# akamiru/bce

Hardware: NVIDIA B200
Metric: compress_MBps_bwt_cse (higher is better)
Workload: dtype u8/u32

## Files before the change

### bce_b200/csrc/api.cu

```cuda
#include <stdarg.h>
#include <stdlib.h>

#include <algorithm>
#include <chrono>
#include <new>

#include "ctx.h"

namespace bce {

static bool g_trace = false;
bool trace_on() { return g_trace; }
static void refresh_trace() {
  const char* v = getenv("BCE_GPU_TRACE");
  g_trace = v && *v && *v != '0';
}

void set_error(Ctx* c, const char* fmt, ...) {
  if (!c) return;
  va_list ap;
  va_start(ap, fmt);
  vsnprintf(c->err, sizeof c->err, fmt, ap);
  va_end(ap);
}

int DevBuf::ensure(Ctx* c, size_t bytes) {
  if (bytes <= cap && p) return BCE_GPU_OK;
  if (p) { cudaFree(p); p = nullptr; cap = 0; }
  size_t want = (bytes + (size_t(1) << 20) - 1) & ~((size_t(1) << 20) - 1);
  cudaError_t e = cudaMalloc(&p, want);
  if (e != cudaSuccess) {
    p = nullptr;
    cudaGetLastError();
    set_error(c, "cudaMalloc(%zu bytes) failed: %s", want, cudaGetErrorString(e));
    return BCE_GPU_E_NOMEM;
  }
  e = cudaMemsetAsync(p, 0, want, c->stream);
  if (e != cudaSuccess) { set_error(c, "cudaMemset failed: %s", cudaGetErrorString(e)); return BCE_GPU_E_CUDA; }
  cap = want;
  return BCE_GPU_OK;
}
void DevBuf::release() {
  if (p) cudaFree(p);
  p = nullptr; cap = 0;
}
int PinnedBuf::ensure(Ctx* c, size_t bytes) {
  if (bytes <= cap && p) return BCE_GPU_OK;
  if (p) { cudaFreeHost(p); p = nullptr; cap = 0; }
  size_t want = (bytes + (size_t(1) << 20) - 1) & ~((size_t(1) << 20) - 1);
  cudaError_t e = cudaHostAlloc(&p, want, cudaHostAllocDefault);
  if (e != cudaSuccess) {
    p = nullptr;
    cudaGetLastError();
    set_error(c, "cudaHostAlloc(%zu bytes) failed: %s", want, cudaGetErrorString(e));
    return BCE_GPU_E_NOMEM;
  }
  cap = want;
  return BCE_GPU_OK;
}
void PinnedBuf::release() {
  if (p) cudaFreeHost(p);
  p = nullptr; cap = 0;
}

int next_tag(Ctx* c) {
  if (++c->desc_tag >= 0x3FFFFFFFu) {
    c->desc_tag = 1;
    if (c->desc.p) cudaMemsetAsync(c->desc.p, 0, c->desc.cap, c->stream);
  }
  return int(c->desc_tag);
}

constexpr size_t kStageChunk = size_t(64) << 20;
bool is_pinned(const void* p) {
  cudaPointerAttributes at;
  if (cudaPointerGetAttributes(&at, p) != cudaSuccess) { cudaGetLastError(); return false; }
  return at.type == cudaMemoryTypeHost;
}
int h2d(Ctx* c, void* dst, const void* src, size_t bytes) {
  if (!bytes) return BCE_GPU_OK;
  if (is_pinned(src) || bytes <= (size_t(1) << 20)) {
    BCE_CUDA(c, cudaMemcpyAsync(dst, src, bytes, cudaMemcpyHostToDevice, c->stream));
    BCE_CUDA(c, cudaStreamSynchronize(c->stream));
    return BCE_GPU_OK;
  }
  BCE_TRY(c->pinned_io.ensure(c, 2 * kStageChunk));
  char* stage = c->pinned_io.as<char>();
  cudaEvent_t done[2] = {c->ev[6], c->ev[7]};
  bool used[2] = {false, false};
  size_t at = 0;
  for (int b = 0; at < bytes; b ^= 1) {
    size_t len = bytes - at < kStageChunk ? bytes - at : kStageChunk;
    if (used[b]) BCE_CUDA(c, cudaEventSynchronize(done[b]));
    memcpy(stage + b * kStageChunk, static_cast<const char*>(src) + at, len);
    BCE_CUDA(c, cudaMemcpyAsync(static_cast<char*>(dst) + at, stage + b * kStageChunk, len,
                                cudaMemcpyHostToDevice, c->stream));
    BCE_CUDA(c, cudaEventRecord(done[b], c->stream));
    used[b] = true;
    at += len;
  }
  BCE_CUDA(c, cudaStreamSynchronize(c->stream));
  return BCE_GPU_OK;
}
int d2h(Ctx* c, void* dst, const void* src, size_t bytes) {
  if (!bytes) return BCE_GPU_OK;
  if (is_pinned(dst) || bytes <= (size_t(1) << 20)) {
    BCE_CUDA(c, cudaMemcpyAsync(dst, src, bytes, cudaMemcpyDeviceToHost, c->stream));
    BCE_CUDA(c, cudaStreamSynchronize(c->stream));
    return BCE_GPU_OK;
  }
  BCE_TRY(c->pinned_io.ensure(c, 2 * kStageChunk));
  char* stage = c->pinned_io.as<char>();
  cudaEvent_t done[2] = {c->ev[6], c->ev[7]};
  size_t at = 0, pending_at[2] = {0, 0}, pending_len[2] = {0, 0};
  bool used[2] = {false, false};
  for (int b = 0; at < bytes; b ^= 1) {
    size_t len = bytes - at < kStageChunk ? bytes - at : kStageChunk;
    if (used[b]) {
      BCE_CUDA(c, cudaEventSynchronize(done[b]));
      memcpy(static_cast<char*>(dst) + pending_at[b], stage + b * kStageChunk, pending_len[b]);
    }
    BCE_CUDA(c, cudaMemcpyAsync(stage + b * kStageChunk, static_cast<const char*>(src) + at, len,
                                cudaMemcpyDeviceToHost, c->stream));
    BCE_CUDA(c, cudaEventRecord(done[b], c->stream));
    used[b] = true; pending_at[b] = at; pending_len[b] = len;
    at += len;
  }
  BCE_CUDA(c, cudaStreamSynchronize(c->stream));
  int order[2] = {0, 1};
  if (used[0] && used[1] && pending_at[1] < pending_at[0]) { order[0] = 1; order[1] = 0; }
  for (int k = 0; k < 2; ++k) {
    int b = order[k];
    if (used[b]) memcpy(static_cast<char*>(dst) + pending_at[b], stage + b * kStageChunk, pending_len[b]);
  }
  return BCE_GPU_OK;
}

size_t scratch_budget(Ctx* c) {
  size_t b = size_t(double(c->total_mem) * 0.70);
  if (c->scratch_limit && c->scratch_limit < b) b = c->scratch_limit;
  return b;
}

static int check_n(Ctx* c, uint32_t n) {
  if (n == 0 || n >= 0x80000000u) { set_error(c, "n = %u outside 1 .. 2^31-1", n); return BCE_GPU_E_ARG; }
  return BCE_GPU_OK;
}

static void begin_call(Ctx* c) {
  refresh_trace();
  c->err[0] = 0;
  cudaSetDevice(c->device);
}

static int upload_text(Ctx* c, const uint8_t* T, uint32_t n) {
  if (c->prefetch_pending) {
    c->prefetch_pending = false;
    const bool arrived = cudaEventQuery(c->ev_prefetch[1]) == cudaSuccess;
    BCE_CUDA(c, cudaEventSynchronize(c->ev_prefetch[1]));
    BCE_TRACE("prefetched input: %s, %s", arrived ? "already on the device" : "still in flight",
              (c->prefetch_src == T && c->prefetch_n == n) ? "adopted" : "another input: discarded");
    if (c->prefetch_src == T && c->prefetch_n == n) {
      float ms = 0;
      BCE_CUDA(c, cudaEventElapsedTime(&ms, c->ev_prefetch[0], c->ev_prefetch[1]));
      c->stats.ms_h2d += ms;
      c->n = n;
      c->text_resident = true;
      c->bwt_resident = false;
      c->ranks_resident = false;
      return BCE_GPU_OK;
    }
  }
  BCE_TRY(c->text.ensure(c, size_t(n) + 128));
  cudaEvent_t a = c->ev[4], b = c->ev[5];
  BCE_CUDA(c, cudaEventRecord(a, c->stream));
  BCE_TRY(h2d(c, c->text.p, T, n));
  BCE_CUDA(c, cudaEventRecord(b, c->stream));
  BCE_CUDA(c, cudaEventSynchronize(b));
  float ms = 0;
  BCE_CUDA(c, cudaEventElapsedTime(&ms, a, b));
  c->stats.ms_h2d += ms;
  c->n = n;
  c->text_resident = true;
  c->bwt_resident = false;
  c->ranks_resident = false;
  return BCE_GPU_OK;
}

static int run_bwt(Ctx* c, uint32_t n, uint32_t* sa_host) {
  cudaEvent_t a = c->ev[4], b = c->ev[5];
  BCE_CUDA(c, cudaEventRecord(a, c->stream));
  BCE_TRY(suffix_sort_bwt(c, n, sa_host));
  BCE_CUDA(c, cudaEventRecord(b, c->stream));
  BCE_CUDA(c, cudaEventSynchronize(b));
  float ms = 0;
  BCE_CUDA(c, cudaEventElapsedTime(&ms, a, b));
  c->stats.ms_bwt_total += ms;
  return BCE_GPU_OK;
}

static int run_cse_begin(Ctx* c, uint32_t n) {
  c->cse_emit_mode_active = int(c->emit_mode);
  cudaEvent_t a = c->ev[4], b = c->ev[5];
  BCE_CUDA(c, cudaEventRecord(a, c->stream));
  BCE_TRY(wavelet_build(c, n));
  BCE_TRY(cse_begin(c, n));
  BCE_CUDA(c, cudaEventRecord(b, c->stream));
  BCE_CUDA(c, cudaEventSynchronize(b));
  float ms = 0;
  BCE_CUDA(c, cudaEventElapsedTime(&ms, a, b));
  c->stats.ms_cse_total += ms;
  return BCE_GPU_OK;
}

static void reset_stats(Ctx* c, uint32_t n) {
  memset(&c->stats, 0, sizeof c->stats);
  c->stats.n = n;
}

}

using bce::Ctx;

extern "C" {

int bce_gpu_abi_version(void) { return BCE_GPU_ABI_VERSION; }

const char* bce_gpu_error_string(int code) {
  switch (code) {
    case BCE_GPU_OK: return "ok";
    case BCE_GPU_E_ARG: return "bad argument";
    case BCE_GPU_E_NOMEM: return "out of memory";
    case BCE_GPU_E_CUDA: return "CUDA failure";
    case BCE_GPU_E_STATE: return "call sequence violated";
    case BCE_GPU_E_FRONTIER: return "CSE frontier exceeded its device memory";
    case BCE_GPU_E_INTERNAL: return "internal consistency check failed";
    case BCE_GPU_E_NODEVICE: return "no usable CUDA device";
    default: return "unknown error";
  }
}

int bce_gpu_open(int device, bce_gpu_ctx** out) {
  if (!out) return BCE_GPU_E_ARG;
  *out = nullptr;
  int count = 0;
  if (cudaGetDeviceCount(&count) != cudaSuccess || count == 0) { cudaGetLastError(); return BCE_GPU_E_NODEVICE; }
  if (device < 0 || device >= count) return BCE_GPU_E_ARG;
  if (cudaSetDevice(device) != cudaSuccess) { cudaGetLastError(); return BCE_GPU_E_NODEVICE; }
  cudaDeviceProp prop;
  if (cudaGetDeviceProperties(&prop, device) != cudaSuccess) { cudaGetLastError(); return BCE_GPU_E_CUDA; }
  if (prop.major < 10 || !prop.cooperativeLaunch) return BCE_GPU_E_NODEVICE;
  Ctx* c = new (std::nothrow) Ctx();
  if (!c) return BCE_GPU_E_NOMEM;
  c->device = device;
  c->sm_count = prop.multiProcessorCount;
  c->total_mem = prop.totalGlobalMem;
  bool ok = cudaStreamCreateWithFlags(&c->stream, cudaStreamNonBlocking) == cudaSuccess &&
            cudaStreamCreateWithFlags(&c->copy_stream, cudaStreamNonBlocking) == cudaSuccess &&
            cudaStreamCreateWithFlags(&c->h2d_stream, cudaStreamNonBlocking) == cudaSuccess &&
            cudaEventCreate(&c->ev_prefetch[0]) == cudaSuccess && cudaEventCreate(&c->ev_prefetch[1]) == cudaSuccess;
  for (int i = 0; ok && i < 8; ++i) ok = cudaEventCreate(&c->ev[i]) == cudaSuccess;
  for (int i = 0; ok && i < 256; ++i) ok = cudaEventCreate(&c->pass_ev[i]) == cudaSuccess;
  if (ok) ok = bce::radix_init_device(c) == BCE_GPU_OK;
  if (ok) ok = c->small.ensure(c, bce::kSmallBytes) == BCE_GPU_OK;
  if (ok) ok = c->pinned_small.ensure(c, bce::kSmallBytes) == BCE_GPU_OK;
  if (ok) ok = cudaStreamSynchronize(c->stream) == cudaSuccess;
  if (!ok) { bce_gpu_close(c); return BCE_GPU_E_CUDA; }
  *out = c;
  return BCE_GPU_OK;
}

void bce_gpu_close(bce_gpu_ctx* h) {
  if (!h) return;
  Ctx* c = static_cast<Ctx*>(h);
  cudaSetDevice(c->device);
  if (c->stream) cudaStreamSynchronize(c->stream);
  bce::cse_destroy(c);
  c->text.release(); c->bwt.release(); c->ranks.release(); c->scratch.release();
  c->small.release(); c->desc.release();
  c->scan_tmp.release(); c->pack_tmp.release();
  c->pinned_small.release(); c->pinned_emit.release(); c->pinned_emit2.release(); c->pinned_io.release();
  c->pinned_many.release(); c->pinned_many2.release();
  for (auto& e : c->ev) if (e) cudaEventDestroy(e);
  for (auto& e : c->pass_ev) if (e) cudaEventDestroy(e);
  if (c->stream) cudaStreamDestroy(c->stream);
  if (c->copy_stream) cudaStreamDestroy(c->copy_stream);
  if (c->h2d_stream) { cudaStreamSynchronize(c->h2d_stream); cudaStreamDestroy(c->h2d_stream); }
  for (auto& e : c->ev_prefetch) if (e) cudaEventDestroy(e);
  delete c;
}

const char* bce_gpu_last_error(const bce_gpu_ctx* h) {
  return h ? static_cast<const Ctx*>(h)->err : "null context";
}

int bce_gpu_get_stats(const bce_gpu_ctx* h, bce_gpu_stats* out) {
  if (!h || !out) return BCE_GPU_E_ARG;
  *out = static_cast<const Ctx*>(h)->stats;
  return BCE_GPU_OK;
}

int bce_gpu_set_scratch_limit(bce_gpu_ctx* h, size_t bytes) {
  if (!h) return BCE_GPU_E_ARG;
  static_cast<Ctx*>(h)->scratch_limit = bytes;
  return BCE_GPU_OK;
}

void* bce_gpu_host_alloc(bce_gpu_ctx* h, size_t bytes) {
  if (!h || !bytes) return nullptr;
  Ctx* c = static_cast<Ctx*>(h);
  cudaSetDevice(c->device);
  void* p = nullptr;
  if (cudaHostAlloc(&p, bytes, cudaHostAllocDefault) != cudaSuccess) {
    cudaGetLastError();
    bce::set_error(c, "cudaHostAlloc(%zu bytes) failed", bytes);
    return nullptr;
  }
  return p;
}

void bce_gpu_host_free(bce_gpu_ctx* h, void* p) {
  if (!h || !p) return;
  cudaSetDevice(static_cast<Ctx*>(h)->device);
  cudaFreeHost(p);
}

int bce_gpu_set_option(bce_gpu_ctx* h, int option, uint64_t value) {
  if (!h) return BCE_GPU_E_ARG;
  Ctx* c = static_cast<Ctx*>(h);
  switch (option) {
    case BCE_GPU_OPT_EMIT_BATCH_BYTES:
      c->emit_batch_bytes = value ? size_t(value) : size_t(1) << 30;
      return BCE_GPU_OK;
    case BCE_GPU_OPT_LOCAL_SORT_MIN:
      c->local_sort_min = value ? uint32_t(value > 0xFFFFFFFFull ? 0xFFFFFFFFull : value) : 1u << 20;
      return BCE_GPU_OK;
    case BCE_GPU_OPT_SLOT_ENTER_NODES:
      c->slot_enter_nodes = value ? value : 2000000;
      return BCE_GPU_OK;
    case BCE_GPU_OPT_MID_ENTER_NODES:
      c->mid_enter_nodes = value ? value : 400000;
      return BCE_GPU_OK;
    case BCE_GPU_OPT_NO_NARROW_KERNELS:
      c->no_narrow_kernels = value != 0;
      return BCE_GPU_OK;
    case BCE_GPU_OPT_RESIDENT_CHECKSUM:
      c->resident_checksum = value != 0;
      return BCE_GPU_OK;
    default:
      set_error(c, "bce_gpu_set_option: unknown option %d", option);
      return BCE_GPU_E_ARG;
  }
}

int bce_gpu_bwt(bce_gpu_ctx* h, const uint8_t* T, uint32_t n, uint8_t* L_out, uint32_t* offset_out,
                uint32_t* SA_out) {
  if (!h || !T) return BCE_GPU_E_ARG;
  Ctx* c = static_cast<Ctx*>(h);
  bce::begin_call(c);
  BCE_TRY(bce::check_n(c, n));
  bce::reset_stats(c, n);
  c->cse_active = false;
  BCE_TRY(bce::upload_text(c, T, n));
  BCE_TRY(bce::run_bwt(c, n, SA_out));
  if (offset_out) *offset_out = c->offset;
  if (L_out) BCE_TRY(bce::d2h(c, L_out, c->bwt.p, n));
  return BCE_GPU_OK;
}

static int load_bwt(Ctx* c, const uint8_t* L, uint32_t n) {
  if (L) {
    BCE_TRY(c->bwt.ensure(c, size_t(n) + 64));
    BCE_TRY(bce::h2d(c, c->bwt.p, L, n));
    c->n = n;
    c->bwt_resident = true;
    c->ranks_resident = false;
  } else if (!c->bwt_resident || c->n != n) {
    bce::set_error(c, "no BWT of length %u resident on the device", n);
    return BCE_GPU_E_STATE;
  }
  return BCE_GPU_OK;
}

int bce_gpu_wavelet(bce_gpu_ctx* h, const uint8_t* L, uint32_t n, uint64_t* const ranks_out[8],
                    uint32_t C_out[8]) {
  if (!h) return BCE_GPU_E_ARG;
  Ctx* c = static_cast<Ctx*>(h);
  bce::begin_call(c);
  BCE_TRY(bce::check_n(c, n));
  if (L) bce::reset_stats(c, n);
  c->cse_active = false;
  BCE_TRY(load_bwt(c, L, n));
  BCE_TRY(bce::wavelet_build(c, n));
  if (C_out) for (int i = 0; i < 8; ++i) C_out[i] = c->C[i];
  if (ranks_out) {
    const size_t words = size_t(n) / 32 + 1;
    for (int j = 0; j < 8; ++j)
      if (ranks_out[j])
        BCE_TRY(bce::d2h(c, ranks_out[j], c->ranks.as<uint64_t>() + size_t(j) * words, words * 8));
  }
  return BCE_GPU_OK;
}

int bce_gpu_cse_begin(bce_gpu_ctx* h, const uint8_t* L, uint32_t n, uint32_t C_out[8]) {
  if (!h) return BCE_GPU_E_ARG;
  Ctx* c = static_cast<Ctx*>(h);
  bce::begin_call(c);
  BCE_TRY(bce::check_n(c, n));
  if (L) bce::reset_stats(c, n);
  c->cse_resident = false;
  BCE_TRY(load_bwt(c, L, n));
  BCE_TRY(bce::run_cse_begin(c, n));
  if (C_out) for (int i = 0; i < 8; ++i) C_out[i] = c->C[i];
  return BCE_GPU_OK;
}

static int next_words(Ctx* c, bce::CseWordBatch* wb, bool pack20 = false) {
  const auto t0 = std::chrono::steady_clock::now();
  BCE_TRY(bce::cse_advance(c, false, wb, pack20));
  c->stats.ms_cse_total += std::chrono::duration<float, std::milli>(std::chrono::steady_clock::now() - t0).count();
  return BCE_GPU_OK;
}

int bce_gpu_cse_next(bce_gpu_ctx* h, bce_cse_batch* out) {
  if (!h || !out) return BCE_GPU_E_ARG;
  Ctx* c = static_cast<Ctx*>(h);
  bce::begin_call(c);
  if (c->cse_active && c->cse_emit_mode_active != BCE_EMIT_RAW) {
    bce::set_error(c, "cse_next: the run emits packed words, use bce_gpu_cse_next_words");
    return BCE_GPU_E_STATE;
  }
  bce::CseWordBatch wb;
  BCE_TRY(next_words(c, &wb));
  for (int i = 0; i < 8; ++i) {
    out->tuples[i] = reinterpret_cast<const bce_tuple*>(wb.words[i]);
    out->count[i] = wb.count[i] / 5;
  }
  out->done = wb.done;
  return BCE_GPU_OK;
}

int bce_gpu_cse_next_words(bce_gpu_ctx* h, bce_cse_words* out) {
  if (!h || !out) return BCE_GPU_E_ARG;
  Ctx* c = static_cast<Ctx*>(h);
  bce::begin_call(c);
  bce::CseWordBatch wb;
  BCE_TRY(next_words(c, &wb));
  for (int i = 0; i < 8; ++i) { out->words[i] = wb.words[i]; out->count[i] = wb.count[i]; }
  out->done = wb.done;
  return BCE_GPU_OK;
}

int bce_gpu_cse_next_words20(bce_gpu_ctx* h, bce_cse_words20* out) {
  if (!h || !out) return BCE_GPU_E_ARG;
  Ctx* c = static_cast<Ctx*>(h);
  bce::begin_call(c);
  if (!c->cse_active || c->cse_emit_mode_active != BCE_EMIT_CODER) {
    bce::set_error(c, "cse_next_words20: needs a run started in BCE_EMIT_CODER mode");
    return BCE_GPU_E_STATE;
  }
  bce::CseWordBatch wb;
  BCE_TRY(next_words(c, &wb, true));
  for (int i = 0; i < 8; ++i) { out->bytes[i] = reinterpret_cast<const uint8_t*>(wb.words[i]); out->count[i] = wb.count[i]; }
  out->done = wb.done;
  return BCE_GPU_OK;
}

int bce_gpu_cse_next_buckets(bce_gpu_ctx* h, bce_scan_buckets* out) {
  if (!h || !out) return BCE_GPU_E_ARG;
  Ctx* c = static_cast<Ctx*>(h);
  bce::begin_call(c);
  if (!c->cse_active || c->cse_emit_mode_active != BCE_EMIT_SCAN) {
    bce::set_error(c, "cse_next_buckets: needs a run started in BCE_EMIT_SCAN mode");
    return BCE_GPU_E_STATE;
  }
  const auto t0 = std::chrono::steady_clock::now();
  BCE_TRY(bce::cse_advance_buckets(c, out));
  c->stats.ms_cse_total += std::chrono::duration<float, std::milli>(std::chrono::steady_clock::now() - t0).count();
  return BCE_GPU_OK;
}

int bce_gpu_set_emit_mode(bce_gpu_ctx* h, int mode, const uint8_t* cfg288) {
  if (!h || mode < BCE_EMIT_RAW || mode > BCE_EMIT_SCAN) return BCE_GPU_E_ARG;
  Ctx* c = static_cast<Ctx*>(h);
  static const uint8_t kDefault[8][32] = {
    {0,0,5,5,5,4,4,4,4,4,4,4,4,4,4,4,4,4,4,4,4,4,4,4,4,4,4,4,4,4,4,0},
    {0,0,5,5,5,4,4,4,4,4,4,4,4,4,4,4,4,4,4,4,4,4,4,4,4,4,4,4,4,4,4,0},
    {0,0,5,5,5,4,4,4,4,4,4,4,4,4,4,4,4,4,4,4,4,4,4,4,4,4,4,3,3,3,3,0},
    {0,0,5,5,5,4,4,4,4,4,4,4,4,4,4,4,4,4,4,4,4,4,3,3,3,3,3,3,3,3,3,0},
    {0,0,5,5,4,4,4,4,4,4,4,4,3,3,3,3,3,3,3,3,3,3,3,3,3,3,3,3,3,3,3,0},
    {0,0,5,5,4,4,4,4,4,4,4,4,3,3,3,3,3,3,3,3,3,3,3,3,3,3,3,3,3,3,3,0},
    {0,0,5,4,4,4,4,4,4,3,3,3,3,3,3,3,3,3,3,3,3,3,3,3,3,3,3,3,3,3,3,0},
    {0,0,4,4,4,4,3,3,3,3,3,3,3,3,3,3,3,3,3,3,3,3,3,3,3,2,2,2,2,2,2,0}};
  c->emit_mode = uint32_t(mode);
  if (cfg288) {
    for (int i = 0; i < 8; ++i)
      for (int k = 0; k < 32; ++k) {
        if (cfg288[i * 32 + k] > 5) { bce::set_error(c, "config: context bits %u > 5", cfg288[i * 32 + k]); return BCE_GPU_E_ARG; }
        c->emit_cfg[i][k] = cfg288[i * 32 + k];
      }
  } else {
    memcpy(c->emit_cfg, kDefault, sizeof kDefault);
  }
  return BCE_GPU_OK;
}

int bce_gpu_compress_front(bce_gpu_ctx* h, const uint8_t* T, uint32_t n, uint32_t* offset_out,
                           uint32_t C_out[8]) {
  if (!h || !T) return BCE_GPU_E_ARG;
  Ctx* c = static_cast<Ctx*>(h);
  bce::begin_call(c);
  BCE_TRY(bce::check_n(c, n));
  bce::reset_stats(c, n);
  c->cse_active = false;
  c->cse_resident = false;
  BCE_TRY(bce::upload_text(c, T, n));
  BCE_TRY(bce::run_bwt(c, n, nullptr));
  BCE_TRY(bce::run_cse_begin(c, n));
  if (offset_out) *offset_out = c->offset;
  if (C_out) for (int i = 0; i < 8; ++i) C_out[i] = c->C[i];
  return BCE_GPU_OK;
}

int bce_gpu_compress_many(bce_gpu_ctx* h, const uint8_t* T, const uint64_t* starts, uint32_t k, bce_many_result* out) {
  if (!h || !T || !starts || !out) return BCE_GPU_E_ARG;
  Ctx* c = static_cast<Ctx*>(h);
  bce::begin_call(c);
  if (k == 0) { bce::set_error(c, "compress_many: no inputs"); return BCE_GPU_E_ARG; }
  uint32_t largest = 0;
  for (uint32_t i = 0; i < k; ++i) {
    if (starts[i + 1] <= starts[i] || starts[i + 1] - starts[i] > BCE_GPU_MANY_MAX_N) {
      bce::set_error(c, "compress_many: input %u: size outside 1 .. %u", i, unsigned(BCE_GPU_MANY_MAX_N));
      return BCE_GPU_E_ARG;
    }
    largest = std::max(largest, uint32_t(starts[i + 1] - starts[i]));
  }
  bce::reset_stats(c, largest);
  if (c->prefetch_pending) {
    BCE_CUDA(c, cudaEventSynchronize(c->ev_prefetch[1]));
    c->prefetch_pending = false;
  }
  c->cse_active = false;
  c->cse_resident = false;
  c->text_resident = c->bwt_resident = c->ranks_resident = false;
  return bce::many_run(c, T, starts, k, out);
}

int bce_gpu_prefetch_input(bce_gpu_ctx* h, const uint8_t* T, uint32_t n) {
  if (!h || !T) return BCE_GPU_E_ARG;
  Ctx* c = static_cast<Ctx*>(h);
  bce::begin_call(c);
  BCE_TRY(bce::check_n(c, n));
  if (!bce::is_pinned(T)) return BCE_GPU_OK;
  if (c->prefetch_pending) { BCE_CUDA(c, cudaEventSynchronize(c->ev_prefetch[1])); c->prefetch_pending = false; }
  BCE_TRY(c->text.ensure(c, size_t(n) + 128));
  BCE_CUDA(c, cudaStreamSynchronize(c->stream));
  BCE_CUDA(c, cudaEventRecord(c->ev_prefetch[0], c->h2d_stream));
  BCE_CUDA(c, cudaMemcpyAsync(c->text.p, T, n, cudaMemcpyHostToDevice, c->h2d_stream));
  BCE_CUDA(c, cudaEventRecord(c->ev_prefetch[1], c->h2d_stream));
  c->text_resident = false;
  c->prefetch_src = T;
  c->prefetch_n = n;
  c->prefetch_pending = true;
  return BCE_GPU_OK;
}

int bce_gpu_stage_input(bce_gpu_ctx* h, const uint8_t* T, uint32_t n) {
  if (!h || !T) return BCE_GPU_E_ARG;
  Ctx* c = static_cast<Ctx*>(h);
  bce::begin_call(c);
  BCE_TRY(bce::check_n(c, n));
  bce::reset_stats(c, n);
  c->cse_active = false;
  return bce::upload_text(c, T, n);
}

int bce_gpu_front_resident(bce_gpu_ctx* h, uint32_t* offset_out, uint64_t* tuples_out) {
  if (!h) return BCE_GPU_E_ARG;
  Ctx* c = static_cast<Ctx*>(h);
  bce::begin_call(c);
  if (!c->text_resident) { bce::set_error(c, "front_resident: no staged input"); return BCE_GPU_E_STATE; }
  const uint32_t n = c->n;
  const float h2d_ms = c->stats.ms_h2d;
  bce::reset_stats(c, n);
  c->stats.ms_h2d = h2d_ms;
  c->cse_active = false;
  c->cse_resident = true;
  BCE_TRY(bce::run_bwt(c, n, nullptr));
  BCE_TRY(bce::run_cse_begin(c, n));
  while (!c->cse_done) {
    cudaEvent_t e0 = c->ev[4], e1 = c->ev[5];
    BCE_CUDA(c, cudaEventRecord(e0, c->stream));
    BCE_TRY(bce::cse_advance(c, true, nullptr));
    BCE_CUDA(c, cudaEventRecord(e1, c->stream));
    BCE_CUDA(c, cudaEventSynchronize(e1));
    float ms = 0;
    BCE_CUDA(c, cudaEventElapsedTime(&ms, e0, e1));
    c->stats.ms_cse_total += ms;
  }
  c->stats.ms_total = c->stats.ms_bwt_total + c->stats.ms_cse_total;
  if (offset_out) *offset_out = c->offset;
  if (tuples_out) *tuples_out = c->emit_mode == BCE_EMIT_RAW ? c->stats.cse_tuples : c->stats.cse_words;
  return BCE_GPU_OK;
}

int bce_gpu_resident_checksum(bce_gpu_ctx* h, uint64_t sum[8], uint64_t wsum[8]) {
  if (!h || !sum || !wsum) return BCE_GPU_E_ARG;
  Ctx* c = static_cast<Ctx*>(h);
  bce::begin_call(c);
  if (!c->cse_resident || !c->cse_done || !c->resident_checksum) {
    bce::set_error(c, "resident_checksum: no finished front_resident run with BCE_GPU_OPT_RESIDENT_CHECKSUM set");
    return BCE_GPU_E_STATE;
  }
  uint64_t acc[16];
  BCE_TRY(bce::d2h(c, acc, c->small.as<char>() + bce::kSmallChecksum, sizeof acc));
  for (int i = 0; i < 8; ++i) { sum[i] = acc[2 * i]; wsum[i] = acc[2 * i + 1]; }
  return BCE_GPU_OK;
}

int bce_gpu_unbwt(bce_gpu_ctx* h, const uint64_t* const ranks[8], uint32_t offset, uint32_t n, uint8_t* out) {
  if (!h || !ranks || !out) return BCE_GPU_E_ARG;
  Ctx* c = static_cast<Ctx*>(h);
  bce::begin_call(c);
  BCE_TRY(bce::check_n(c, n));
  if (offset >= n) { bce::set_error(c, "offset %u >= n %u", offset, n); return BCE_GPU_E_ARG; }
  bce::reset_stats(c, n);
  c->cse_active = false;
  const size_t words = size_t(n) / 32 + 1;
  BCE_TRY(c->ranks.ensure(c, 8 * words * 8));
  for (int j = 0; j < 8; ++j) {
    if (!ranks[j]) return BCE_GPU_E_ARG;
    BCE_TRY(bce::h2d(c, c->ranks.as<uint64_t>() + size_t(j) * words, ranks[j], words * 8));
    uint64_t w = ranks[j][n / 32];
    uint32_t ones = uint32_t(w) + uint32_t(__builtin_popcount(uint32_t(w >> 32) & ((1u << (n % 32)) - 1u)));
    c->C[(j + 1) & 7] = n - ones;
  }
  c->n = n;
  c->ranks_resident = true;
  c->bwt_resident = false;
  c->text_resident = false;
  return bce::unbwt_run(c, offset, n, out);
}

}
```

### bce_b200/csrc/common.cuh

```cuda
#pragma once

#include <cuda_runtime.h>
#include <stdint.h>
#include <stdio.h>
#include <string.h>

#include "../../include/bce_gpu.h"

namespace bce {

constexpr int kSMsB200 = 148;

struct Ctx;
void set_error(Ctx* c, const char* fmt, ...);
bool trace_on();
#define BCE_TRACE(...) do { if (bce::trace_on()) { fprintf(stderr, "[bce_gpu] " __VA_ARGS__); fputc('\n', stderr); fflush(stderr); } } while (0)

#define BCE_CUDA(ctx, call)                                                         \
  do {                                                                              \
    cudaError_t e__ = (call);                                                       \
    if (e__ != cudaSuccess) {                                                       \
      bce::set_error((ctx), "%s:%d %s -> %s", __FILE__, __LINE__, #call,            \
                     cudaGetErrorString(e__));                                      \
      return (e__ == cudaErrorMemoryAllocation) ? BCE_GPU_E_NOMEM : BCE_GPU_E_CUDA; \
    }                                                                               \
  } while (0)

#define BCE_TRY(expr)            \
  do {                           \
    int rc__ = (expr);           \
    if (rc__ != BCE_GPU_OK) return rc__; \
  } while (0)

struct DevBuf {
  void* p = nullptr;
  size_t cap = 0;
  int ensure(Ctx* c, size_t bytes);
  void release();
  template <class T> T* as() const { return reinterpret_cast<T*>(p); }
};

struct PinnedBuf {
  void* p = nullptr;
  size_t cap = 0;
  int ensure(Ctx* c, size_t bytes);
  void release();
  template <class T> T* as() const { return reinterpret_cast<T*>(p); }
};

struct Carver {
  char* base;
  size_t off = 0, cap;
  Carver(void* b, size_t c) : base(reinterpret_cast<char*>(b)), cap(c) {}
  template <class T> T* take(size_t count) {
    size_t bytes = (count * sizeof(T) + 255) & ~size_t(255);
    if (off + bytes > cap) { off = cap + 1; return nullptr; }
    T* r = reinterpret_cast<T*>(base + off);
    off += bytes;
    return r;
  }
  bool ok() const { return off <= cap; }
  static size_t need(size_t count, size_t elem) { return (count * elem + 255) & ~size_t(255); }
};

#ifdef __CUDACC__

__device__ __forceinline__ unsigned lane_id() { return threadIdx.x & 31; }
__device__ __forceinline__ unsigned lanemask_lt() {
  unsigned m;
  asm("mov.u32 %0, %%lanemask_lt;" : "=r"(m));
  return m;
}

__device__ __forceinline__ uint64_t bswap64(uint64_t v) {
  const uint32_t lo = uint32_t(v), hi = uint32_t(v >> 32);
  return (uint64_t(__byte_perm(lo, 0, 0x0123)) << 32) | __byte_perm(hi, 0, 0x0123);
}

__device__ __forceinline__ uint64_t window_key(const uint64_t* T64, uint32_t i) {
  const uint64_t a = bswap64(T64[i >> 3]), b = bswap64(T64[(i >> 3) + 1]);
  const uint32_t sh = (i & 7u) * 8;
  return sh ? (a << sh) | (b >> (64 - sh)) : a;
}

constexpr uint32_t kDescAgg = 1, kDescPrefix = 2;
__device__ __forceinline__ uint64_t desc_pack(uint32_t tag, uint32_t status, uint32_t value) {
  return (uint64_t(tag & 0x3FFFFFFFu) << 34) | (uint64_t(status) << 32) | value;
}
__device__ __forceinline__ uint32_t desc_tag(uint64_t w) { return uint32_t(w >> 34); }
__device__ __forceinline__ uint32_t desc_status(uint64_t w) { return uint32_t(w >> 32) & 3u; }
__device__ __forceinline__ void desc_store(uint64_t* p, uint64_t v) {
  asm volatile("st.relaxed.gpu.global.u64 [%0], %1;" ::"l"(p), "l"(v) : "memory");
}
__device__ __forceinline__ uint64_t desc_load(const uint64_t* p) {
  uint64_t v;
  asm volatile("ld.relaxed.gpu.global.u64 %0, [%1];" : "=l"(v) : "l"(p) : "memory");
  return v;
}

constexpr uint32_t kSpinBudget = 1u << 18;
#ifndef BCE_SPIN_HOT
#define BCE_SPIN_HOT 64
#define BCE_SPIN_SLEEP 20
#endif
__device__ __forceinline__ uint64_t desc_wait(const uint64_t* p, uint32_t tag, uint32_t* err) {
  uint64_t w = desc_load(p);
  uint32_t spins = 0;
  while (desc_tag(w) != (tag & 0x3FFFFFFFu)) {
    if (++spins > kSpinBudget) {
      atomicExch(err, 1u);
      return desc_pack(tag, kDescPrefix, 0);
    }
    if (spins > BCE_SPIN_HOT) __nanosleep(BCE_SPIN_SLEEP);
    w = desc_load(p);
  }
  return w;
}

__device__ __forceinline__ uint32_t lookback_serial(uint64_t* desc, uint32_t stride, uint32_t tile,
                                                    uint32_t tag, uint32_t agg, uint32_t* err) {
  if (tile == 0) {
    desc_store(desc, desc_pack(tag, kDescPrefix, agg));
    return 0;
  }
  desc_store(desc + size_t(tile) * stride, desc_pack(tag, kDescAgg, agg));
  #ifndef BCE_LB_BATCH
#define BCE_LB_BATCH 2
#endif
  constexpr int kBatch = BCE_LB_BATCH;
  uint32_t excl = 0;
  uint32_t t = tile;
  bool done = false;
  while (!done && t > 0) {
    uint64_t w[kBatch];
    const uint32_t nb = t < uint32_t(kBatch) ? t : uint32_t(kBatch);
#pragma unroll
    for (int k = 0; k < kBatch; ++k)
      if (uint32_t(k) < nb) w[k] = desc_load(desc + size_t(t - 1 - k) * stride);
#pragma unroll
    for (int k = 0; k < kBatch; ++k) {
      if (!done && uint32_t(k) < nb) {
        uint64_t v = w[k];
        if (desc_tag(v) != (tag & 0x3FFFFFFFu)) v = desc_wait(desc + size_t(t - 1 - k) * stride, tag, err);
        excl += uint32_t(v);
        if (desc_status(v) == kDescPrefix) done = true;
      }
    }
    t -= nb;
  }
  desc_store(desc + size_t(tile) * stride, desc_pack(tag, kDescPrefix, excl + agg));
  return excl;
}

__device__ __forceinline__ uint32_t lookback_warp(uint64_t* desc, uint32_t tile, uint32_t first,
                                                  uint32_t tag, uint32_t agg, uint32_t* err) {
  const unsigned lane = lane_id();
  if (tile == first) {
    if (lane == 0) desc_store(desc + tile, desc_pack(tag, kDescPrefix, agg));
    return 0;
  }
  if (lane == 0) desc_store(desc + tile, desc_pack(tag, kDescAgg, agg));
  uint32_t excl = 0;
  int64_t base = int64_t(tile) - 1;
  for (;;) {
    int64_t t = base - lane;
    bool inside = t >= int64_t(first);
    uint64_t w = inside ? desc_wait(desc + t, tag, err) : desc_pack(tag, kDescPrefix, 0);
    unsigned pm = __ballot_sync(0xffffffffu, desc_status(w) == kDescPrefix);
    uint32_t v = uint32_t(w);
    if (pm) {
      unsigned stop = __ffs(pm) - 1;
      if (lane > stop) v = 0;
      excl += __reduce_add_sync(0xffffffffu, v);
      break;
    }
    excl += __reduce_add_sync(0xffffffffu, v);
    base -= 32;
  }
  if (lane == 0) desc_store(desc + tile, desc_pack(tag, kDescPrefix, excl + agg));
  return excl;
}

__device__ __forceinline__ uint32_t lookback_warp_max(uint64_t* desc, uint32_t tile, uint32_t first,
                                                      uint32_t tag, uint32_t agg, uint32_t* err) {
  const unsigned lane = lane_id();
  if (tile == first) {
    if (lane == 0) desc_store(desc + tile, desc_pack(tag, kDescPrefix, agg));
    return 0;
  }
  if (lane == 0) desc_store(desc + tile, desc_pack(tag, agg ? kDescPrefix : kDescAgg, agg));
  uint32_t excl = 0;
  int64_t base = int64_t(tile) - 1;
  for (;;) {
    int64_t t = base - lane;
    bool inside = t >= int64_t(first);
    uint64_t w = inside ? desc_wait(desc + t, tag, err) : desc_pack(tag, kDescPrefix, 0);
    unsigned pm = __ballot_sync(0xffffffffu, desc_status(w) == kDescPrefix);
    uint32_t v = uint32_t(w);
    if (pm) {
      unsigned stop = __ffs(pm) - 1;
      if (lane > stop) v = 0;
      excl = max(excl, __reduce_max_sync(0xffffffffu, v));
      break;
    }
    excl = max(excl, __reduce_max_sync(0xffffffffu, v));
    base -= 32;
  }
  if (lane == 0 && !agg) desc_store(desc + tile, desc_pack(tag, kDescPrefix, excl));
  return excl;
}

template <int B>
__device__ __forceinline__ uint32_t lookback_resolve_wide(uint64_t* desc, uint32_t tile, uint32_t first,
                                                          uint32_t tag, uint32_t agg, uint32_t* err) {
  const unsigned lane = lane_id();
  uint32_t excl = 0;
  int64_t base = int64_t(tile) - 1;
  for (;;) {
    uint64_t w[B];
#pragma unroll
    for (int k = 0; k < B; ++k) {
      const int64_t t = base - (k * 32 + int(lane));
      w[k] = t >= int64_t(first) ? desc_load(desc + t) : desc_pack(tag, kDescPrefix, 0);
    }
#pragma unroll
    for (int k = 0; k < B; ++k) {
      const int64_t t = base - (k * 32 + int(lane));
      if (t >= int64_t(first) && desc_tag(w[k]) != (tag & 0x3FFFFFFFu)) w[k] = desc_wait(desc + t, tag, err);
    }
    bool done = false;
#pragma unroll
    for (int k = 0; k < B; ++k) {
      if (!done) {
        const unsigned pm = __ballot_sync(0xffffffffu, desc_status(w[k]) == kDescPrefix);
        uint32_t v = uint32_t(w[k]);
        if (pm) {
          const unsigned stop = __ffs(pm) - 1;
          if (lane > stop) v = 0;
          done = true;
        }
        excl += __reduce_add_sync(0xffffffffu, v);
      }
    }
    if (done) break;
    base -= 32 * B;
  }
  if (lane == 0) desc_store(desc + tile, desc_pack(tag, kDescPrefix, excl + agg));
  return excl;
}

template <int B>
__device__ __forceinline__ uint32_t lookback_warp_wide(uint64_t* desc, uint32_t tile, uint32_t first,
                                                       uint32_t tag, uint32_t agg, uint32_t* err) {
  if (tile == first) {
    if (lane_id() == 0) desc_store(desc + tile, desc_pack(tag, kDescPrefix, agg));
    return 0;
  }
  if (lane_id() == 0) desc_store(desc + tile, desc_pack(tag, kDescAgg, agg));
  return lookback_resolve_wide<B>(desc, tile, first, tag, agg, err);
}

template <class T, int THREADS>
__device__ __forceinline__ T block_exclusive_scan_sparse(T v, T* scratch, T& total, bool active) {
  constexpr int NW = THREADS / 32;
  const unsigned lane = lane_id(), warp = threadIdx.x >> 5;
  T inc = v;
  if (active) {
#pragma unroll
    for (int d = 1; d < 32; d <<= 1) {
      T o = __shfl_up_sync(0xffffffffu, inc, d);
      if (lane >= unsigned(d)) inc += o;
    }
  }
  if (lane == 31) scratch[warp] = active ? inc : T(0);
  __syncthreads();
  T woff = 0;
  if (active) {
    T winc = lane < unsigned(NW) ? scratch[lane] : T(0);
#pragma unroll
    for (int d = 1; d < NW; d <<= 1) {
      T o = __shfl_up_sync(0xffffffffu, winc, d);
      if (lane >= unsigned(d)) winc += o;
    }
    total = __shfl_sync(0xffffffffu, winc, NW - 1);
    const T before = __shfl_sync(0xffffffffu, winc, warp ? warp - 1 : 0);
    woff = warp ? before : T(0);
  }
  __syncthreads();
  return woff + inc - v;
}

template <class T, int THREADS>
__device__ __forceinline__ T block_exclusive_scan(T v, T* scratch, T& total) {
  constexpr int NW = THREADS / 32;
  const unsigned lane = lane_id(), warp = threadIdx.x >> 5;
  T inc = v;
#pragma unroll
  for (int d = 1; d < 32; d <<= 1) {
    T o = __shfl_up_sync(0xffffffffu, inc, d);
    if (lane >= unsigned(d)) inc += o;
  }
  if (lane == 31) scratch[warp] = inc;
  __syncthreads();
  T woff = 0, tot = 0;
#pragma unroll
  for (int w = 0; w < NW; ++w) {
    T s = scratch[w];
    if (unsigned(w) < warp) woff += s;
    tot += s;
  }
  __syncthreads();
  total = tot;
  return woff + inc - v;
}

#endif

}
```

### bce_b200/csrc/ctx.h

```cpp
#pragma once

#include <stdlib.h>

#include "common.cuh"

struct bce_gpu_ctx {};

namespace bce {

constexpr int kMaxSortRounds = 48;

inline size_t exp_env(const char* name, size_t dflt) {
#ifdef BCE_GPU_EXPERIMENTS
  const char* v = getenv(name);
  if (v && *v) return size_t(strtoull(v, nullptr, 10));
#else
  (void)name;
#endif
  return dflt;
}

struct CseDeviceState;

struct Ctx : bce_gpu_ctx {
  int device = 0;
  int sm_count = 0;
  size_t total_mem = 0;
  cudaStream_t stream = nullptr;
  cudaStream_t copy_stream = nullptr;
  cudaStream_t h2d_stream = nullptr;
  cudaEvent_t ev_prefetch[2] = {};
  const uint8_t* prefetch_src = nullptr;
  uint32_t prefetch_n = 0;
  bool prefetch_pending = false;
  cudaEvent_t ev[8] = {};
  cudaEvent_t pass_ev[256] = {};
  int pass_ev_n = 0;
  char err[512] = {0};
  size_t scratch_limit = 0;

  DevBuf text;
  DevBuf bwt;
  DevBuf ranks;
  DevBuf scratch;
  DevBuf small;
  DevBuf desc;
  PinnedBuf pinned_small;
  PinnedBuf pinned_emit;
  PinnedBuf pinned_emit2;
  PinnedBuf pinned_io;
  DevBuf scan_tmp;
  DevBuf pack_tmp;
  PinnedBuf pinned_many;
  PinnedBuf pinned_many2;
  int many_flip = 0;

  uint32_t desc_tag = 0;

  size_t emit_batch_bytes = size_t(1) << 30;
  uint32_t local_sort_min = 1u << 20;
  bool resident_checksum = false;
  uint64_t slot_enter_nodes = 2000000;
  uint64_t mid_enter_nodes = 400000;
  bool no_narrow_kernels = false;

  uint32_t n = 0;
  bool text_resident = false;
  bool bwt_resident = false;
  bool ranks_resident = false;
  uint32_t offset = 0;
  uint32_t C[8] = {};

  uint32_t emit_mode = 0;
  uint8_t emit_cfg[8][32] = {};
  bool cse_resident = false;
  int cse_emit_mode_active = 0;

  bool cse_active = false;
  bool cse_done = false;
  struct CseHost* cse = nullptr;

  bce_gpu_stats stats = {};
};

constexpr size_t kSmallHist = 0;
constexpr size_t kSmallBase = kSmallHist + 8 * 256 * 4;
constexpr size_t kSmallTicket = kSmallBase + 8 * 256 * 4;
constexpr size_t kSmallErr = kSmallTicket + 64;
constexpr size_t kSmallRerankTicket = kSmallErr + 64;
constexpr size_t kSmallRerankTotals = kSmallRerankTicket + 64;
constexpr size_t kSmallWavelet = kSmallRerankTotals + 64;
constexpr size_t kSmallCse = kSmallWavelet + 2048;
constexpr size_t kSmallUnbwt = kSmallCse + 1024;
constexpr size_t kSmallChecksum = 44 * 1024;
constexpr size_t kSmallRadixCursor = 52 * 1024;
constexpr size_t kSmallPartHist = 48 * 1024;
constexpr size_t kSmallPartCursor = kSmallPartHist + 1024;
constexpr size_t kSmallBytes = 64 * 1024;

struct RadixHistSource {
  const uint8_t* window_text = nullptr;
  const uint32_t* dev_hist = nullptr;
  bool stable_first = false;
};
int radix_sort_pairs(Ctx* c, uint64_t* keyA, uint64_t* keyB, uint32_t* valA, uint32_t* valB,
                     uint32_t m, const int* shifts, int npass, uint64_t** out_k, uint32_t** out_v,
                     int* passes_run, const RadixHistSource* src = nullptr);
constexpr int kRadixMaxPasses = 8;
struct RadixShifts { int s[kRadixMaxPasses]; };
size_t radix_desc_words(uint32_t m);

int suffix_sort_bwt(Ctx* c, uint32_t n, uint32_t* sa_host_or_null);
int wavelet_build(Ctx* c, uint32_t n);
void byte_hist_launch(Ctx* c, const uint8_t* L, uint32_t n, uint32_t* d_hist);
int cse_begin(Ctx* c, uint32_t n);
struct CseWordBatch { const uint32_t* words[8]; size_t count[8]; int done; };
int cse_advance(Ctx* c, bool resident, CseWordBatch* out, bool pack20 = false);
int cse_advance_buckets(Ctx* c, bce_scan_buckets* out);
void cse_destroy(Ctx* c);
int unbwt_run(Ctx* c, uint32_t offset, uint32_t n, uint8_t* out_host);
int many_run(Ctx* c, const uint8_t* T, const uint64_t* starts, uint32_t k, bce_many_result* out);

int next_tag(Ctx* c);
bool is_pinned(const void* p);
int h2d(Ctx* c, void* dst, const void* src, size_t bytes);
int d2h(Ctx* c, void* dst, const void* src, size_t bytes);
int radix_init_device(Ctx* c);
size_t scratch_budget(Ctx* c);

}
```

### bce_b200/csrc/radix_sort.cu

```cuda
#include <math.h>

#include "ctx.h"

namespace bce {

constexpr int RS_MIN_TILE = 2048;
constexpr int RS_MAX_PASSES = kRadixMaxPasses;
constexpr int kRadixThreads = 256, kRadixItems = 24;
constexpr size_t kRadixSmem = size_t(kRadixThreads) * kRadixItems * 12 + size_t(kRadixThreads / 32) * 1024;
constexpr size_t kRadixUnorderedSmem = size_t(256) * kRadixItems * 12;

size_t radix_desc_words(uint32_t m) { return (size_t(m) / RS_MIN_TILE + 1) * 256; }

constexpr int RH_THREADS = 256;
constexpr int RH_WARPS = RH_THREADS / 32;

__global__ void __launch_bounds__(RH_THREADS) radix_hist_kernel(const uint64_t* __restrict__ keys, uint32_t m,
                                                                int npass, RadixShifts sh,
                                                                uint32_t* __restrict__ hist) {
  extern __shared__ uint32_t rh_smem[];
  const unsigned tid = threadIdx.x, lane = tid & 31, warp = tid >> 5;
  for (int i = tid; i < RH_WARPS * npass * 256; i += RH_THREADS) rh_smem[i] = 0;
  __syncthreads();
  uint32_t* h = rh_smem + size_t(warp) * npass * 256;
  const uint32_t stride = gridDim.x * RH_THREADS;
  const uint32_t rounds = (m + stride - 1) / stride;
  uint32_t i = blockIdx.x * RH_THREADS + tid;
  for (uint32_t r = 0; r < rounds; ++r, i += stride) {
    const bool in = i < m;
    const uint64_t k = in ? keys[i] : 0;
    const unsigned active = __ballot_sync(0xffffffffu, in);
    if (active == 0xffffffffu) {
      for (int p = 0; p < npass; ++p) {
        const uint32_t d = uint32_t(k >> sh.s[p]) & 255u;
        int same;
        __match_all_sync(0xffffffffu, d, &same);
        if (same) { if (lane == 0) h[p * 256 + d] += 32; }
        else atomicAdd(&h[p * 256 + d], 1u);
        __syncwarp();
      }
    } else if (in) {
      for (int p = 0; p < npass; ++p) atomicAdd(&h[p * 256 + (uint32_t(k >> sh.s[p]) & 255u)], 1u);
    }
  }
  __syncthreads();
  for (int j = tid; j < npass * 256; j += RH_THREADS) {
    uint32_t v = 0;
#pragma unroll
    for (int w = 0; w < RH_WARPS; ++w) v += rh_smem[size_t(w) * npass * 256 + j];
    if (v) atomicAdd(&hist[j], v);
  }
}

struct RadixPass {
  const uint64_t* kin;
  const uint32_t* vin;
  uint64_t* kout;
  uint32_t* vout;
  uint32_t m;
  int shift;
  const uint32_t* base;
  uint64_t* desc;
  uint32_t* ticket;
  uint32_t tag;
  uint32_t* err;
};

template <int RS_THREADS, int RS_ITEMS, int MIN_CTAS, bool BALLOT = false>
__global__ void __launch_bounds__(RS_THREADS, MIN_CTAS) radix_onesweep_kernel(RadixPass p) {
  constexpr int RS_TILE = RS_THREADS * RS_ITEMS;
  constexpr int RS_WARPS = RS_THREADS / 32;
  extern __shared__ __align__(16) unsigned char rs_smem[];
  uint64_t* s_keys = reinterpret_cast<uint64_t*>(rs_smem);
  uint32_t* s_vals = reinterpret_cast<uint32_t*>(rs_smem + size_t(RS_TILE) * 8);
  uint32_t (*s_whist)[256] = reinterpret_cast<uint32_t (*)[256]>(rs_smem + size_t(RS_TILE) * 12);
  __shared__ uint32_t s_goff[256];
  __shared__ uint32_t s_dstart[256];
  __shared__ uint32_t s_scan[RS_WARPS];
  __shared__ uint32_t s_tile;

  const unsigned tid = threadIdx.x, lane = tid & 31, warp = tid >> 5;
  if (tid == 0) s_tile = atomicAdd(p.ticket, 1u);
  for (int i = tid; i < RS_WARPS * 256; i += RS_THREADS) (&s_whist[0][0])[i] = 0;
  __syncthreads();
  const uint32_t tile = s_tile;
  const uint32_t tile_base = tile * uint32_t(RS_TILE);
  const uint32_t valid = min(uint32_t(RS_TILE), p.m - tile_base);
  const uint32_t wbase = tile_base + warp * (32 * RS_ITEMS);

  uint64_t key[RS_ITEMS];
  uint32_t val[RS_ITEMS];
  uint32_t pos[RS_ITEMS];
#pragma unroll
  for (int k = 0; k < RS_ITEMS; ++k) {
    uint32_t idx = wbase + k * 32 + lane;
    bool in = idx < p.m;
    key[k] = in ? p.kin[idx] : ~0ull;
    val[k] = (in && p.vin) ? p.vin[idx] : 0u;
  }
#pragma unroll
  for (int k = 0; k < RS_ITEMS; ++k) {
    uint32_t d = uint32_t(key[k] >> p.shift) & 255u;
unsigned peers;
    if (BALLOT) {
      peers = 0xffffffffu;
#pragma unroll
      for (int b = 0; b < 8; ++b) {
        const unsigned v = __ballot_sync(0xffffffffu, (d >> b) & 1u);
        peers &= ((d >> b) & 1u) ? v : ~v;
      }
    } else {
      peers = __match_any_sync(0xffffffffu, d);
    }
    unsigned leader = __ffs(peers) - 1;
    uint32_t before = 0;
    if (lane == leader) {
      before = s_whist[warp][d];
      s_whist[warp][d] = before + __popc(peers);
    }
    before = __shfl_sync(0xffffffffu, before, leader);
    pos[k] = before + __popc(peers & lanemask_lt());
    __syncwarp();
  }
  __syncthreads();

  {
    const uint32_t d = tid;
    uint32_t sum = 0;
    if (d < 256u) {
#pragma unroll
    for (int w = 0; w < RS_WARPS; ++w) {
      uint32_t c = s_whist[w][d];
      s_whist[w][d] = sum;
      sum += c;
    }
    }
    uint32_t tot;
    uint32_t dstart = block_exclusive_scan<uint32_t, RS_THREADS>(sum, s_scan, tot);
    if (d < 256u) {
      s_dstart[d] = dstart;
      uint32_t publish = (d == 255u) ? sum - (uint32_t(RS_TILE) - valid) : sum;
      uint32_t excl = lookback_serial(p.desc + d, 256u, tile, p.tag, publish, p.err);
      s_goff[d] = p.base[d] + excl - dstart;
    }
  }
  __syncthreads();

#pragma unroll
  for (int k = 0; k < RS_ITEMS; ++k) {
    uint32_t d = uint32_t(key[k] >> p.shift) & 255u;
    pos[k] += s_dstart[d] + s_whist[warp][d];
    s_keys[pos[k]] = key[k];
    s_vals[pos[k]] = val[k];
  }
  __syncthreads();
  for (uint32_t j = tid; j < valid; j += RS_THREADS) {
    uint64_t k64 = s_keys[j];
    uint32_t d = uint32_t(k64 >> p.shift) & 255u;
    uint32_t g = s_goff[d] + j;
    p.kout[g] = k64;
    if (p.vout) p.vout[g] = s_vals[j];
  }
}


template <int RS_ITEMS, int MIN_CTAS, bool FROM_TEXT>
__global__ void __launch_bounds__(256, MIN_CTAS) radix_unordered_kernel(RadixPass p, uint32_t* __restrict__ cursor,
                                                                        const uint8_t* __restrict__ text) {
  constexpr int RS_THREADS = 256;
  constexpr int RS_TILE = RS_THREADS * RS_ITEMS;
  extern __shared__ __align__(16) unsigned char ru_smem[];
  uint64_t* s_keys = reinterpret_cast<uint64_t*>(ru_smem);
  uint32_t* s_vals = reinterpret_cast<uint32_t*>(ru_smem + size_t(RS_TILE) * 8);
  __shared__ uint32_t s_cnt[256], s_start[256], s_goff[256];
  __shared__ uint32_t s_scan[RS_THREADS / 32];

  const unsigned tid = threadIdx.x, lane = tid & 31, warp = tid >> 5;
  s_cnt[tid] = 0;
  __syncthreads();
  const uint32_t tile_base = blockIdx.x * uint32_t(RS_TILE);
  const uint32_t valid = min(uint32_t(RS_TILE), p.m - tile_base);
  const uint32_t wbase = tile_base + warp * (32 * RS_ITEMS);
  const bool has_vals = FROM_TEXT || p.vin != nullptr;

  uint64_t key[RS_ITEMS];
  uint32_t val[RS_ITEMS];
  uint32_t pos[RS_ITEMS / 2];
#pragma unroll
  for (int k = 0; k < RS_ITEMS; ++k) {
    const uint32_t idx = wbase + k * 32 + lane;
    const bool in = idx < p.m;
    if (FROM_TEXT) {
      key[k] = in ? window_key(reinterpret_cast<const uint64_t*>(text), idx) : 0ull;
      val[k] = idx;
    } else {
      key[k] = in ? p.kin[idx] : 0ull;
      val[k] = (in && has_vals) ? p.vin[idx] : 0u;
    }
  }
#pragma unroll
  for (int k = 0; k < RS_ITEMS; ++k) {
    const bool in = wbase + k * 32 + lane < p.m;
    const uint32_t at = in ? atomicAdd(&s_cnt[uint32_t(key[k] >> p.shift) & 255u], 1u) : 0u;
    pos[k / 2] = (k & 1) ? (pos[k / 2] | (at << 16)) : at;
  }
  __syncthreads();
  {
    const uint32_t c = s_cnt[tid];
    uint32_t tot;
    const uint32_t st = block_exclusive_scan<uint32_t, RS_THREADS>(c, s_scan, tot);
    s_start[tid] = st;
    s_goff[tid] = p.base[tid] + (c ? atomicAdd(&cursor[tid], c) : 0u) - st;
  }
  __syncthreads();
#pragma unroll
  for (int k = 0; k < RS_ITEMS; ++k) {
    if (wbase + k * 32 + lane < p.m) {
      const uint32_t at = s_start[uint32_t(key[k] >> p.shift) & 255u] + ((pos[k / 2] >> ((k & 1) * 16)) & 0xFFFFu);
      s_keys[at] = key[k];
      s_vals[at] = val[k];
    }
  }
  __syncthreads();
  for (uint32_t j = tid; j < valid; j += RS_THREADS) {
    const uint64_t k64 = s_keys[j];
    const uint32_t g = s_goff[uint32_t(k64 >> p.shift) & 255u] + j;
    p.kout[g] = k64;
    if (has_vals) p.vout[g] = s_vals[j];
  }
}

constexpr double kBallotAboveDistinct = 24;

int radix_sort_pairs(Ctx* c, uint64_t* keyA, uint64_t* keyB, uint32_t* valA, uint32_t* valB,
                     uint32_t m, const int* shifts, int npass, uint64_t** out_k, uint32_t** out_v,
                     int* passes_run, const RadixHistSource* src) {
  *out_k = keyA;
  *out_v = valA;
  if (passes_run) *passes_run = 0;
  if (m <= 1 || npass <= 0) return BCE_GPU_OK;
  if (npass > RS_MAX_PASSES) return BCE_GPU_E_ARG;

  char* small = c->small.as<char>();
  uint32_t* d_hist = reinterpret_cast<uint32_t*>(small + kSmallHist);
  uint32_t* d_base = reinterpret_cast<uint32_t*>(small + kSmallBase);
  uint32_t* d_ticket = reinterpret_cast<uint32_t*>(small + kSmallTicket);
  uint32_t* d_err = reinterpret_cast<uint32_t*>(small + kSmallErr);
  uint32_t* h_hist = c->pinned_small.as<uint32_t>();

  BCE_TRY(c->desc.ensure(c, radix_desc_words(m) * sizeof(uint64_t)));

  RadixShifts sh;
  for (int i = 0; i < RS_MAX_PASSES; ++i) sh.s[i] = i < npass ? shifts[i] : 0;
  const uint8_t* window_text = src ? src->window_text : nullptr;
  const uint32_t* dev_hist = src ? src->dev_hist : nullptr;
  if (dev_hist == d_hist) BCE_CUDA(c, cudaMemsetAsync(d_base, 0, kSmallErr - kSmallBase, c->stream));
  else BCE_CUDA(c, cudaMemsetAsync(d_hist, 0, kSmallErr, c->stream));
  if (dev_hist) {
    BCE_CUDA(c, cudaMemcpyAsync(h_hist, dev_hist, npass * 256 * 4, cudaMemcpyDeviceToHost, c->stream));
    BCE_CUDA(c, cudaStreamSynchronize(c->stream));
  } else if (window_text) {
    byte_hist_launch(c, window_text, m, d_hist);
    c->stats.gpu_launches++;
    BCE_CUDA(c, cudaGetLastError());
    BCE_CUDA(c, cudaMemcpyAsync(h_hist, d_hist, 256 * 4, cudaMemcpyDeviceToHost, c->stream));
    BCE_CUDA(c, cudaStreamSynchronize(c->stream));
    for (int p = npass - 1; p >= 0; --p)
      for (int d = 0; d < 256; ++d) h_hist[p * 256 + d] = h_hist[d];
  } else {
    const size_t hsmem = size_t(RH_WARPS) * npass * 256 * 4;
    uint64_t hb64 = (uint64_t(m) + 255) / 256, hbmax = uint64_t(c->sm_count) * 3;
    int hb = int(hb64 < hbmax ? hb64 : hbmax);
    radix_hist_kernel<<<hb, RH_THREADS, hsmem, c->stream>>>(keyA, m, npass, sh, d_hist);
    c->stats.gpu_launches++;
    BCE_CUDA(c, cudaGetLastError());
    BCE_CUDA(c, cudaMemcpyAsync(h_hist, d_hist, npass * 256 * 4, cudaMemcpyDeviceToHost, c->stream));
    BCE_CUDA(c, cudaStreamSynchronize(c->stream));
  }

  bool run[RS_MAX_PASSES];
  uint32_t* h_base = h_hist + RS_MAX_PASSES * 256;
  for (int p = 0; p < npass; ++p) {
    run[p] = true;
    uint32_t acc = 0;
    for (int d = 0; d < 256; ++d) {
      uint32_t cnt = h_hist[p * 256 + d];
      if (cnt == m) run[p] = false;
      h_base[p * 256 + d] = acc;
      acc += cnt;
    }
  }
  BCE_CUDA(c, cudaMemcpyAsync(d_base, h_base, npass * 256 * 4, cudaMemcpyHostToDevice, c->stream));

  uint64_t* kin = keyA; uint64_t* kout = keyB;
  uint32_t* vin = valA; uint32_t* vout = valB;
  constexpr int RS_THREADS = kRadixThreads, RS_TILE = kRadixThreads * kRadixItems;
  constexpr size_t rs_smem = kRadixSmem;
  const uint32_t tiles = (m + RS_TILE - 1) / RS_TILE;
  const bool unordered_first = !(src && src->stable_first);
  int ran = 0;
  for (int p = 0; p < npass; ++p) {
    if (!run[p]) continue;
    RadixPass a;
    a.kin = kin; a.vin = vin; a.kout = kout; a.vout = vout;
    a.m = m; a.shift = shifts[p];
    a.base = d_base + p * 256;
    a.desc = c->desc.as<uint64_t>();
    a.ticket = d_ticket + p;
    a.tag = uint32_t(next_tag(c));
    a.err = d_err;
    const bool timed = c->pass_ev_n + 2 <= 256;
    if (timed) cudaEventRecord(c->pass_ev[c->pass_ev_n], c->stream);
    if (ran == 0 && unordered_first) {
      uint32_t* d_cursor = reinterpret_cast<uint32_t*>(small + kSmallRadixCursor);
      BCE_CUDA(c, cudaMemsetAsync(d_cursor, 0, 256 * 4, c->stream));
      constexpr int UI = kRadixItems;
      constexpr size_t usmem = kRadixUnorderedSmem;
      const uint32_t ugrid = (m + 256 * UI - 1) / (256 * UI);
      if (window_text) radix_unordered_kernel<UI, 2, true><<<ugrid, 256, usmem, c->stream>>>(a, d_cursor, window_text);
      else radix_unordered_kernel<UI, 2, false><<<ugrid, 256, usmem, c->stream>>>(a, d_cursor, nullptr);
    } else {
      double distinct = 0;
      for (int d = 0; d < 256; ++d) {
        const double q = double(h_hist[p * 256 + d]) / double(m);
        if (q > 0) distinct += 1.0 - pow(1.0 - q, 32.0);
      }
      const bool context_sorted = window_text && ran >= 2;
      const bool ballot = distinct > kBallotAboveDistinct && !context_sorted;
      if (ballot) radix_onesweep_kernel<kRadixThreads, kRadixItems, 2, true><<<tiles, RS_THREADS, rs_smem, c->stream>>>(a);
      else radix_onesweep_kernel<kRadixThreads, kRadixItems, 2, false><<<tiles, RS_THREADS, rs_smem, c->stream>>>(a);
    }
    if (timed) { cudaEventRecord(c->pass_ev[c->pass_ev_n + 1], c->stream); c->pass_ev_n += 2; }
    c->stats.gpu_launches++;
    c->stats.radix_launches++;
    c->stats.radix_elems += m;
    BCE_CUDA(c, cudaGetLastError());
    uint64_t* tk = kin; kin = kout; kout = tk;
    uint32_t* tv = vin; vin = vout; vout = tv;
    ++ran;
  }
  *out_k = kin;
  *out_v = vin;
  if (passes_run) *passes_run = ran;
  return BCE_GPU_OK;
}


int radix_init_device(Ctx* c) {
  BCE_CUDA(c, cudaFuncSetAttribute(radix_hist_kernel, cudaFuncAttributeMaxDynamicSharedMemorySize, RH_WARPS * RS_MAX_PASSES * 1024));
  BCE_CUDA(c, cudaFuncSetAttribute(radix_onesweep_kernel<kRadixThreads, kRadixItems, 2, true>, cudaFuncAttributeMaxDynamicSharedMemorySize, int(kRadixSmem)));
  BCE_CUDA(c, cudaFuncSetAttribute(radix_onesweep_kernel<kRadixThreads, kRadixItems, 2, false>, cudaFuncAttributeMaxDynamicSharedMemorySize, int(kRadixSmem)));
  BCE_CUDA(c, cudaFuncSetAttribute(radix_unordered_kernel<kRadixItems, 2, false>, cudaFuncAttributeMaxDynamicSharedMemorySize, int(kRadixUnorderedSmem)));
  BCE_CUDA(c, cudaFuncSetAttribute(radix_unordered_kernel<kRadixItems, 2, true>, cudaFuncAttributeMaxDynamicSharedMemorySize, int(kRadixUnorderedSmem)));
  return BCE_GPU_OK;
}

}
```

### bce_b200/csrc/suffix_sort.cu

```cuda
#include <algorithm>
#include <utility>

#include "ctx.h"
#include "local_sort.cuh"

namespace bce {

__global__ void pad_cyclic_kernel(uint8_t* T, uint32_t n) {
  uint32_t k = threadIdx.x;
  if (k < 64) T[size_t(n) + k] = T[k % n];
}

constexpr int PK_ROWS = 8;

__global__ void __launch_bounds__(256) pack_keys_kernel(const uint8_t* __restrict__ T, uint32_t n,
                                                        uint64_t* __restrict__ keys,
                                                        uint32_t* __restrict__ idx) {
  const uint64_t* T64 = reinterpret_cast<const uint64_t*>(T);
  const uint32_t tile = blockIdx.x * (256 * PK_ROWS);
#pragma unroll
  for (int r = 0; r < PK_ROWS; ++r) {
    const uint32_t i = tile + r * 256 + threadIdx.x;
    if (i < n) {
      keys[i] = window_key(T64, i);
      idx[i] = i;
    }
  }
}

constexpr int RR_THREADS = 256;
constexpr int RR_WARPS = RR_THREADS / 32;
constexpr int RR_ROWS = 16;
constexpr int RR_WCHUNK = 32 * RR_ROWS;
constexpr int RR_TILE = RR_WARPS * RR_WCHUNK;
constexpr int RR_LOOKBACK = 4;

struct RerankArgs {
  const uint64_t* key;
  const uint32_t* idx;
  const uint32_t* sapos;
  uint32_t m;
  uint32_t* sa;
  uint32_t* rnk;
  uint64_t* pairs;
  uint32_t* part_cursor;
  int part_shift;
  uint32_t* idx_out;
  uint32_t* sapos_out;
  uint32_t* gd_out;
  uint32_t* totals;
  uint64_t* desc;
  uint32_t tiles;
  uint32_t* ticket;
  uint32_t tag;
  uint32_t* err;
};

__global__ void __launch_bounds__(RR_THREADS) rerank_kernel(RerankArgs a) {
  __shared__ uint32_t s_whead[RR_WARPS], s_wsurv[RR_WARPS], s_wshead[RR_WARPS];
  __shared__ uint32_t s_tile;
  __shared__ uint32_t s_carry[3];
  __shared__ uint32_t s_bcnt[256], s_bstart[256], s_gbase[256];
  __shared__ uint32_t s_bscan[RR_WARPS];
  __shared__ uint64_t s_stage[RR_TILE];

  const unsigned tid = threadIdx.x, lane = tid & 31, warp = tid >> 5;
  if (tid == 0) s_tile = atomicAdd(a.ticket, 1u);
  s_bcnt[tid] = 0;
  __syncthreads();
  const uint32_t tile = s_tile;
  const uint32_t wbase = tile * RR_TILE + warp * RR_WCHUNK;
  const bool binned = a.pairs != nullptr;

  uint64_t key[RR_ROWS];
  uint32_t idx[RR_ROWS], sap[RR_ROWS];
#pragma unroll
  for (int k = 0; k < RR_ROWS; ++k) {
    const uint32_t q = wbase + k * 32 + lane;
    const bool in = q < a.m;
    key[k] = in ? a.key[q] : 0;
    idx[k] = in ? a.idx[q] : 0;
    sap[k] = in ? (a.sapos ? a.sapos[q] : q) : 0;
  }
  uint32_t bpos[RR_ROWS / 2];
  if (binned) {
#pragma unroll
    for (int k = 0; k < RR_ROWS; ++k) {
      const uint32_t q = wbase + k * 32 + lane;
      const uint32_t at = q < a.m ? atomicAdd(&s_bcnt[(idx[k] >> a.part_shift) & 255u], 1u) : 0u;
      bpos[k / 2] = (k & 1) ? (bpos[k / 2] | (at << 16)) : at;
    }
  }
  const uint64_t key_before = (wbase > 0 && wbase - 1 < a.m) ? a.key[wbase - 1] : 0;
  const uint64_t key_after = (wbase + RR_WCHUNK < a.m) ? a.key[wbase + RR_WCHUNK] : 0;

  uint32_t H[RR_ROWS];
#pragma unroll
  for (int k = 0; k < RR_ROWS; ++k) {
    const uint32_t q = wbase + k * 32 + lane;
    const uint64_t up = __shfl_up_sync(0xffffffffu, key[k], 1);
    const uint64_t wrap = k ? __shfl_sync(0xffffffffu, key[k ? k - 1 : 0], 31) : key_before;
    const uint64_t prev = lane ? up : wrap;
    H[k] = __ballot_sync(0xffffffffu, q < a.m && (q == 0 || key[k] != prev));
  }
  const bool after_is_head = (wbase + RR_WCHUNK >= a.m) ||
                             (key_after != __shfl_sync(0xffffffffu, key[RR_ROWS - 1], 31));
  auto masks = [&](int k, uint32_t& S, uint32_t& SH, uint32_t& L) {
    const uint32_t rowbase = wbase + k * 32;
    const uint32_t valid = rowbase >= a.m ? 0u : a.m - rowbase;
    const uint32_t in_mask = valid >= 32u ? 0xFFFFFFFFu : (1u << valid) - 1u;
    const uint32_t next_first = k + 1 < RR_ROWS ? (H[k + 1 < RR_ROWS ? k + 1 : k] & 1u) : (after_is_head ? 1u : 0u);
    uint32_t nh = (H[k] >> 1) | (next_first << 31);
    if (valid <= 32u) nh |= valid ? ~((1u << (valid - 1u)) - 1u) : 0xFFFFFFFFu;
    L = H[k] & nh & in_mask;
    S = in_mask & ~L;
    SH = H[k] & ~L;
  };
  uint32_t wsurv = 0, wshead = 0, whead = 0;
#pragma unroll
  for (int k = 0; k < RR_ROWS; ++k) {
    uint32_t S, SH, L;
    masks(k, S, SH, L);
    wsurv += __popc(S);
    wshead += __popc(SH);
    if (H[k]) whead = wbase + k * 32 + (31 - __clz(H[k])) + 1;
  }
  if (lane == 0) { s_whead[warp] = whead; s_wsurv[warp] = wsurv; s_wshead[warp] = wshead; }
  __syncthreads();
  if (binned) {
    const uint32_t c = s_bcnt[tid];
    uint32_t tot;
    s_bstart[tid] = block_exclusive_scan<uint32_t, RR_THREADS>(c, s_bscan, tot);
    s_gbase[tid] = c ? atomicAdd(&a.part_cursor[tid], c) : 0u;
  }
  uint32_t head_before = 0, surv_before = 0, shead_before = 0, tile_head = 0, tile_surv = 0, tile_shead = 0;
#pragma unroll
  for (int w = 0; w < RR_WARPS; ++w) {
    const uint32_t hv = s_whead[w], sv = s_wsurv[w], shv = s_wshead[w];
    if (unsigned(w) < warp) { head_before = max(head_before, hv); surv_before += sv; shead_before += shv; }
    tile_head = max(tile_head, hv);
    tile_surv += sv;
    tile_shead += shv;
  }
  if (warp < 3) {
    uint64_t* d = a.desc + size_t(warp) * a.tiles;
    uint32_t v;
    if (warp == 0) v = lookback_warp_max(d, tile, 0u, a.tag, tile_head, a.err);
    else if (warp == 1) v = lookback_warp_wide<RR_LOOKBACK>(d, tile, 0u, a.tag, tile_surv, a.err);
    else v = lookback_warp_wide<RR_LOOKBACK>(d, tile, 0u, a.tag, tile_shead, a.err);
    if (lane == 0) s_carry[warp] = v;
  }
  __syncthreads();
  uint32_t run_head = max(head_before, s_carry[0]);
  uint32_t out_at = s_carry[1] + surv_before;
  uint32_t gd_run = s_carry[2] + shead_before;

#pragma unroll
  for (int k = 0; k < RR_ROWS; ++k) {
    const uint32_t q = wbase + k * 32 + lane;
    uint32_t S, SH, L;
    masks(k, S, SH, L);
    const uint32_t le = lanemask_lt() | (1u << lane);
    const uint32_t hm = H[k] & le;
    const uint32_t my_head = hm ? wbase + k * 32 + (31 - __clz(hm)) + 1 : run_head;
    if (q < a.m) {
      const uint32_t rank = sap[k] - (q - (my_head - 1));
      if ((L >> lane) & 1u) a.sa[sap[k]] = idx[k];
      if (binned) s_stage[s_bstart[(idx[k] >> a.part_shift) & 255u] + ((bpos[k / 2] >> ((k & 1) * 16)) & 0xFFFFu)] = (uint64_t(idx[k]) << 32) | rank;
      else a.rnk[idx[k]] = rank;
      if ((S >> lane) & 1u) {
        const uint32_t at = out_at + __popc(S & lanemask_lt());
        a.idx_out[at] = idx[k];
        a.sapos_out[at] = sap[k];
        a.gd_out[at] = gd_run + __popc(SH & le) - 1;
      }
    }
    if (H[k]) run_head = wbase + k * 32 + (31 - __clz(H[k])) + 1;
    out_at += __popc(S);
    gd_run += __popc(SH);
  }
  if (binned) {
    __syncthreads();
    const uint32_t tile_valid = min(uint32_t(RR_TILE), a.m - tile * RR_TILE);
    for (uint32_t j = tid; j < tile_valid; j += RR_THREADS) {
      const uint64_t pr = s_stage[j];
      const uint32_t d = (uint32_t(pr >> 32) >> a.part_shift) & 255u;
      a.pairs[s_gbase[d] + (j - s_bstart[d])] = pr;
    }
  }
  if (tile == a.tiles - 1 && tid == RR_THREADS - 1) {
    a.totals[0] = s_carry[1] + tile_surv;
    a.totals[1] = s_carry[2] + tile_shead;
  }
}

__global__ void __launch_bounds__(256) partition_cursor_kernel(const uint32_t* __restrict__ hist, uint32_t* __restrict__ cursor) {
  __shared__ uint32_t s_scan[8];
  uint32_t tot;
  cursor[threadIdx.x] = block_exclusive_scan<uint32_t, 256>(hist[threadIdx.x], s_scan, tot);
}

__global__ void __launch_bounds__(256) scatter_ranks_kernel(const uint64_t* __restrict__ pairs, uint32_t m,
                                                            uint32_t* __restrict__ rnk) {
  uint32_t q = blockIdx.x * blockDim.x + threadIdx.x;
  if (q >= m) return;
  const uint64_t p = pairs[q];
  rnk[uint32_t(p >> 32)] = uint32_t(p);
}

struct RekeyHist {
  RadixShifts sh;
  int npass;
  uint32_t* hist;
  uint32_t* phist;
  int pshift;
};
constexpr int RK_THREADS = 256;
constexpr int RK_ITEMS = 4;

__device__ __forceinline__ void hist_add(uint32_t* set, uint32_t d, bool full_warp, unsigned lane) {
  if (full_warp) {
    const uint32_t d0 = __shfl_sync(0xffffffffu, d, 0);
    if (__all_sync(0xffffffffu, d == d0)) {
      if (lane == 0) atomicAdd(&set[d0], 32u);
      return;
    }
  }
  atomicAdd(&set[d], 1u);
}

__global__ void __launch_bounds__(RK_THREADS) rekey_kernel(const uint32_t* __restrict__ idx,
                                                           const uint32_t* __restrict__ gd,
                                                           const uint32_t* __restrict__ rnk, uint32_t m,
                                                           uint32_t n, uint32_t h, int tiebreak,
                                                           uint64_t* __restrict__ key, RekeyHist rh) {
  __shared__ uint32_t s_hist[2][kRadixMaxPasses + 1][256];
  const unsigned tid = threadIdx.x, lane = tid & 31, warp = tid >> 5;
  for (int i = tid; i < 2 * (kRadixMaxPasses + 1) * 256; i += RK_THREADS) (&s_hist[0][0][0])[i] = 0;
  __syncthreads();
  uint32_t (*set)[256] = s_hist[warp & 1];
  const uint32_t chunk = RK_THREADS * RK_ITEMS;
  for (uint64_t base = uint64_t(blockIdx.x) * chunk; base < m; base += uint64_t(gridDim.x) * chunk) {
    uint32_t i[RK_ITEMS], second[RK_ITEMS], g[RK_ITEMS];
    bool in[RK_ITEMS];
#pragma unroll
    for (int u = 0; u < RK_ITEMS; ++u) {
      const uint64_t q = base + uint64_t(u) * RK_THREADS + tid;
      in[u] = q < m;
      i[u] = in[u] ? idx[q] : 0u;
    }
#pragma unroll
    for (int u = 0; u < RK_ITEMS; ++u) {
      if (tiebreak) {
        second[u] = i[u];
      } else {
        uint64_t j = uint64_t(i[u]) + h;
        if (j >= n) j -= n;
        second[u] = in[u] ? rnk[j] : 0u;
      }
    }
#pragma unroll
    for (int u = 0; u < RK_ITEMS; ++u) {
      const uint64_t q = base + uint64_t(u) * RK_THREADS + tid;
      g[u] = in[u] ? gd[q] : 0u;
    }
#pragma unroll
    for (int u = 0; u < RK_ITEMS; ++u) {
      const uint64_t q = base + uint64_t(u) * RK_THREADS + tid;
      const uint64_t k = (uint64_t(g[u]) << 32) | second[u];
      if (in[u]) key[q] = k;
      const bool full_warp = __ballot_sync(0xffffffffu, in[u]) == 0xffffffffu;
      if (in[u] || full_warp) {
        for (int p = 0; p < rh.npass; ++p) hist_add(set[p], uint32_t(k >> rh.sh.s[p]) & 255u, full_warp, lane);
        if (rh.phist) hist_add(set[kRadixMaxPasses], (i[u] >> rh.pshift) & 255u, full_warp, lane);
      }
    }
  }
  __syncthreads();
  for (int j = tid; j < rh.npass * 256; j += RK_THREADS) {
    const uint32_t v = s_hist[0][j >> 8][j & 255] + s_hist[1][j >> 8][j & 255];
    if (v) atomicAdd(&rh.hist[j], v);
  }
  if (rh.phist) {
    const uint32_t v = s_hist[0][kRadixMaxPasses][tid] + s_hist[1][kRadixMaxPasses][tid];
    if (v) atomicAdd(&rh.phist[tid], v);
  }
}

__global__ void __launch_bounds__(256) bwt_gather_kernel(const uint8_t* __restrict__ T,
                                                         const uint32_t* __restrict__ sa, uint32_t n,
                                                         uint8_t* __restrict__ L) {
  uint32_t r4 = (blockIdx.x * blockDim.x + threadIdx.x) * 4;
  if (r4 >= n) return;
  uint32_t out = 0;
#pragma unroll
  for (int j = 0; j < 4; ++j) {
    uint32_t r = r4 + j;
    if (r < n) {
      uint32_t s = sa[r];
      uint32_t c = T[s ? s - 1 : n - 1];
      out |= c << (8 * j);
    }
  }
  if (r4 + 4 <= n) *reinterpret_cast<uint32_t*>(L + r4) = out;
  else for (int j = 0; r4 + j < n; ++j) L[r4 + j] = uint8_t(out >> (8 * j));
}

constexpr int BG_THREADS = 256, BG_ITEMS = 16, BG_TILE = BG_THREADS * BG_ITEMS;
__global__ void bwt_cursor_kernel(uint32_t* cursor, int shift) { cursor[threadIdx.x] = threadIdx.x << shift; }

__global__ void __launch_bounds__(BG_THREADS) bwt_bin_kernel(const uint8_t* __restrict__ T, const uint32_t* __restrict__ rnk,
                                                             uint32_t n, int shift, uint32_t* __restrict__ cursor,
                                                             uint32_t* __restrict__ pairs) {
  __shared__ uint32_t s_cnt[256], s_start[256], s_gbase[256];
  __shared__ uint32_t s_scan[BG_THREADS / 32];
  __shared__ uint32_t s_stage[BG_TILE];
  __shared__ uint8_t s_bin[BG_TILE];
  const unsigned tid = threadIdx.x;
  const uint32_t base = blockIdx.x * BG_TILE;
  s_cnt[tid] = 0;
  __syncthreads();
  uint32_t word[BG_ITEMS], pos[BG_ITEMS];
  const uint32_t mask = (1u << shift) - 1u;
#pragma unroll
  for (int k = 0; k < BG_ITEMS; ++k) {
    const uint32_t i = base + k * BG_THREADS + tid;
    word[k] = pos[k] = 0;
    if (i < n) {
      const uint32_t r = rnk[i];
      const uint32_t byte = T[i ? i - 1 : n - 1];
      const uint32_t bin = r >> shift;
      pos[k] = atomicAdd(&s_cnt[bin], 1u) | (bin << 16);
      word[k] = ((r & mask) << 8) | byte;
    }
  }
  __syncthreads();
  uint32_t tot;
  const uint32_t mine = s_cnt[tid];
  s_start[tid] = block_exclusive_scan<uint32_t, BG_THREADS>(mine, s_scan, tot);
  if (mine) s_gbase[tid] = atomicAdd(&cursor[tid], mine);
  __syncthreads();
#pragma unroll
  for (int k = 0; k < BG_ITEMS; ++k)
    if (base + k * BG_THREADS + tid < n) {
      const uint32_t at = s_start[pos[k] >> 16] + (pos[k] & 0xFFFFu);
      s_stage[at] = word[k];
      s_bin[at] = uint8_t(pos[k] >> 16);
    }
  __syncthreads();
  const uint32_t valid = min(uint32_t(BG_TILE), n - base);
  for (uint32_t j = tid; j < valid; j += BG_THREADS) {
    const uint32_t bin = s_bin[j];
    pairs[s_gbase[bin] + (j - s_start[bin])] = s_stage[j];
  }
}

__global__ void __launch_bounds__(256) bwt_scatter_kernel(const uint32_t* __restrict__ pairs, uint32_t n, int shift,
                                                          uint8_t* __restrict__ L) {
  for (uint32_t j = blockIdx.x * 256u + threadIdx.x; j < n; j += gridDim.x * 256u) {
    const uint32_t p = pairs[j];
    L[((j >> shift) << shift) + (p >> 8)] = uint8_t(p);
  }
}

static inline int bits_for(uint32_t values) {
  int b = 0;
  while (b < 32 && (uint64_t(1) << b) < values) ++b;
  return b ? b : 1;
}

static inline int top_byte_shift(uint32_t n) { return std::max(0, bits_for(n) - 8); }

constexpr uint32_t kBinnedRanksMinSlots = 8u << 20;
constexpr size_t kBinnedRanksMinBytes = size_t(64) << 20;
constexpr uint32_t kBinnedBwtMinN = 8u << 20;
constexpr uint32_t kLocalFallbackDiv = 4;

struct RoundPlan {
  int shifts[kRadixMaxPasses];
  int np = 0;
  bool tiebreak = false;
  bool binned = false;
  int part_shift = 0;
};

static RoundPlan plan_round(int round, uint32_t m, uint32_t n, uint64_t h, uint32_t groups) {
  RoundPlan p;
  p.binned = m >= kBinnedRanksMinSlots && size_t(n) * 4 > kBinnedRanksMinBytes;
  p.part_shift = top_byte_shift(n);
  if (round == 0) {
    for (int s = 0; s < 64; s += 8) p.shifts[p.np++] = s;
    return p;
  }
  p.tiebreak = h >= n;
  const int nbits = bits_for(n), gbits = bits_for(groups);
  for (int s = 0; s < nbits; s += 8) p.shifts[p.np++] = s;
  for (int s = 0; s < gbits && p.np < kRadixMaxPasses; s += 8) p.shifts[p.np++] = 32 + s;
  return p;
}

struct SortReadback {
  uint32_t totals[2];
  uint32_t err;
  uint32_t fb_total;
  uint32_t offset;
  uint32_t bins[256];
};
constexpr size_t kPinnedSortReadback = 32 * 1024;

struct SortBuffers {
  uint64_t* key[2];
  uint32_t* idx[2];
  uint32_t* sapos[2];
  uint32_t* gd[2];
  uint32_t* sa;
  uint32_t* rnk;
  uint64_t* fb_key[2];
  uint32_t* fb_idx[2];
  uint32_t* fb_slot;
  uint32_t *lt_pre, *lt_suf, *lt_cnt, *lt_off;
  uint32_t *err, *ticket, *totals, *fb_total, *hist, *part_hist, *part_cursor;
  SortReadback* rb;

  void next_round() {
    std::swap(idx[0], idx[1]);
    std::swap(sapos[0], sapos[1]);
    std::swap(gd[0], gd[1]);
  }
};

static int carve(Ctx* c, uint32_t n, SortBuffers& b) {
  const size_t N = n, FB = N / kLocalFallbackDiv + 1, LT = N / LS_TILE + 2;
  const size_t need = 2 * Carver::need(N, 8) + 8 * Carver::need(N, 4) + 2 * Carver::need(FB, 8) +
                      3 * Carver::need(FB, 4) + 4 * Carver::need(LT, 4) + 4096;
  BCE_TRY(c->scratch.ensure(c, need));
  Carver cv(c->scratch.p, c->scratch.cap);
  for (auto& k : b.key) k = cv.take<uint64_t>(N);
  for (auto& v : b.idx) v = cv.take<uint32_t>(N);
  b.sa = cv.take<uint32_t>(N);
  b.rnk = cv.take<uint32_t>(N);
  for (auto& v : b.sapos) v = cv.take<uint32_t>(N);
  for (auto& v : b.gd) v = cv.take<uint32_t>(N);
  for (auto& k : b.fb_key) k = cv.take<uint64_t>(FB);
  for (auto& v : b.fb_idx) v = cv.take<uint32_t>(FB);
  b.fb_slot = cv.take<uint32_t>(FB);
  b.lt_pre = cv.take<uint32_t>(LT);
  b.lt_suf = cv.take<uint32_t>(LT);
  b.lt_cnt = cv.take<uint32_t>(LT);
  b.lt_off = cv.take<uint32_t>(LT);
  if (!cv.ok()) { set_error(c, "suffix sort: scratch carve failed"); return BCE_GPU_E_NOMEM; }

  char* small = c->small.as<char>();
  b.err = reinterpret_cast<uint32_t*>(small + kSmallErr);
  b.ticket = reinterpret_cast<uint32_t*>(small + kSmallRerankTicket);
  b.totals = reinterpret_cast<uint32_t*>(small + kSmallRerankTotals);
  b.fb_total = b.totals + 3;
  b.hist = reinterpret_cast<uint32_t*>(small + kSmallHist);
  b.part_hist = reinterpret_cast<uint32_t*>(small + kSmallPartHist);
  b.part_cursor = reinterpret_cast<uint32_t*>(small + kSmallPartCursor);
  b.rb = reinterpret_cast<SortReadback*>(c->pinned_small.as<char>() + kPinnedSortReadback);
  return BCE_GPU_OK;
}

static int lap(Ctx* c, float& acc) {
  BCE_CUDA(c, cudaEventRecord(c->ev[1], c->stream));
  BCE_CUDA(c, cudaEventSynchronize(c->ev[1]));
  float ms = 0;
  BCE_CUDA(c, cudaEventElapsedTime(&ms, c->ev[0], c->ev[1]));
  acc += ms;
  BCE_CUDA(c, cudaEventRecord(c->ev[0], c->stream));
  return BCE_GPU_OK;
}

static int sort_round(Ctx* c, SortBuffers& b, const RoundPlan& p, int round, uint32_t m, uint32_t n, uint64_t h) {
  cudaStream_t st = c->stream;
  bce_gpu_stats& S = c->stats;
  const uint8_t* T = c->text.as<uint8_t>();
  const uint32_t second_h = uint32_t(p.tiebreak ? 0 : h);
  const uint32_t ltiles = (m + LS_TILE - 1) / LS_TILE;
  bool local = false;
  if (round > 0 && m >= c->local_sort_min) {
    ls_classify_kernel<<<(ltiles + 255) / 256, 256, 0, st>>>(b.gd[0], m, ltiles, b.lt_pre, b.lt_suf, b.lt_cnt);
    ls_scan_kernel<<<1, 1024, 0, st>>>(b.lt_cnt, ltiles, b.lt_off, b.fb_total);
    S.gpu_launches += 2;
    BCE_CUDA(c, cudaGetLastError());
    BCE_CUDA(c, cudaMemcpyAsync(&b.rb->fb_total, b.fb_total, 4, cudaMemcpyDeviceToHost, st));
    BCE_CUDA(c, cudaStreamSynchronize(st));
    BCE_TRACE("local sort round %d: %u of %u slots in groups that cross a tile boundary", round, b.rb->fb_total, m);
    local = b.rb->fb_total <= m / kLocalFallbackDiv;
  }
  const uint32_t m_fb = local ? b.rb->fb_total : 0;
  if (local) {
    if (p.binned) {
      BCE_CUDA(c, cudaMemsetAsync(b.part_hist, 0, 256 * 4, st));
      const uint32_t want = (m + 255) / 256, most = uint32_t(c->sm_count) * 8;
      ls_idx_hist_kernel<<<want < most ? want : most, 256, 0, st>>>(b.idx[0], m, p.part_shift, b.part_hist);
      S.gpu_launches++;
    }
    BCE_TRY(lap(c, S.ms_rekey));
  } else if (round > 0) {
    RekeyHist rh;
    for (int i = 0; i < kRadixMaxPasses; ++i) rh.sh.s[i] = i < p.np ? p.shifts[i] : 0;
    rh.npass = p.np;
    rh.hist = b.hist;
    rh.phist = p.binned ? b.part_hist : nullptr;
    rh.pshift = p.part_shift;
    BCE_CUDA(c, cudaMemsetAsync(b.hist, 0, kRadixMaxPasses * 256 * 4, st));
    BCE_CUDA(c, cudaMemsetAsync(b.part_hist, 0, 256 * 4, st));
    const uint32_t chunk = RK_THREADS * RK_ITEMS;
    const uint32_t want = (m + chunk - 1) / chunk, most = uint32_t(c->sm_count) * 8;
    rekey_kernel<<<want < most ? want : most, RK_THREADS, 0, st>>>(b.idx[0], b.gd[0], b.rnk, m, n, second_h,
                                                                   p.tiebreak ? 1 : 0, b.key[0], rh);
    S.gpu_launches++;
    BCE_CUDA(c, cudaGetLastError());
    BCE_TRY(lap(c, S.ms_rekey));
  }
  BCE_TRACE("sort round %d m=%u h=%llu tiebreak=%d passes<=%d", round, m, (unsigned long long)h, int(p.tiebreak), p.np);
  int ran = 0;
  if (local) {
    LocalSortArgs la;
    la.vin = b.idx[0]; la.gd = b.gd[0]; la.rnk = b.rnk;
    la.n = n; la.h = second_h; la.tiebreak = p.tiebreak ? 1 : 0;
    la.kout = b.key[1]; la.vout = b.idx[1]; la.m = m;
    la.pre = b.lt_pre; la.suf = b.lt_suf; la.off = b.lt_off;
    la.fb_key = b.fb_key[0]; la.fb_idx = b.fb_idx[0]; la.fb_slot = b.fb_slot;
    ls_sort_kernel<<<ltiles, LS_THREADS, 0, st>>>(la);
    S.gpu_launches++;
    BCE_CUDA(c, cudaGetLastError());
    if (m_fb) {
      uint64_t* sk; uint32_t* sv; int fran = 0;
      BCE_TRY(radix_sort_pairs(c, b.fb_key[0], b.fb_key[1], b.fb_idx[0], b.fb_idx[1], m_fb, p.shifts, p.np, &sk, &sv,
                               &fran, nullptr));
      ls_place_kernel<<<(m_fb + 255) / 256, 256, 0, st>>>(sk, sv, b.fb_slot, m_fb, b.key[1], b.idx[1]);
      S.gpu_launches++;
      BCE_CUDA(c, cudaGetLastError());
    }
    std::swap(b.key[0], b.key[1]);
    std::swap(b.idx[0], b.idx[1]);
    ran = p.np;
    S.sort_local_elems += m;
    S.sort_fallback_elems += m_fb;
  } else {
    RadixHistSource src;
    if (round == 0) src.window_text = T; else src.dev_hist = b.hist;
    uint64_t* ks; uint32_t* vs;
    BCE_TRY(radix_sort_pairs(c, b.key[0], b.key[1], b.idx[0], b.idx[1], m, p.shifts, p.np, &ks, &vs, &ran, &src));
    if (ks != b.key[0]) {
      std::swap(b.key[0], b.key[1]);
      std::swap(b.idx[0], b.idx[1]);
    }
    if (round == 0 && ran == 0) {
      pack_keys_kernel<<<(n + 256 * PK_ROWS - 1) / (256 * PK_ROWS), 256, 0, st>>>(T, n, b.key[0], b.idx[0]);
      S.gpu_launches++;
    }
  }
  BCE_TRY(lap(c, S.ms_radix));
  S.sort_m[round] = m;
  S.sort_passes[round] = uint32_t(ran);
  S.sort_radix_passes[round] = local ? 0u : uint32_t(ran);
  S.sort_rounds = uint32_t(round + 1);
  return BCE_GPU_OK;
}

static int rerank_round(Ctx* c, SortBuffers& b, const RoundPlan& p, int round, uint32_t m, uint32_t n,
                        uint32_t* m_next, uint32_t* groups) {
  cudaStream_t st = c->stream;
  bce_gpu_stats& S = c->stats;
  RerankArgs a;
  a.key = b.key[0]; a.idx = b.idx[0]; a.sapos = round ? b.sapos[0] : nullptr; a.m = m;
  a.sa = b.sa; a.rnk = b.rnk;
  a.pairs = nullptr; a.part_cursor = nullptr; a.part_shift = p.part_shift;
  if (p.binned) {
    if (round == 0) {
      for (uint32_t d = 0; d < 256; ++d) {
        const uint64_t lo = uint64_t(d) << p.part_shift, hi = uint64_t(d + 1) << p.part_shift;
        b.rb->bins[d] = uint32_t(lo >= n ? 0 : (hi < n ? hi : n) - lo);
      }
      BCE_CUDA(c, cudaMemcpyAsync(b.part_hist, b.rb->bins, 256 * 4, cudaMemcpyHostToDevice, st));
    }
    partition_cursor_kernel<<<1, 256, 0, st>>>(b.part_hist, b.part_cursor);
    S.gpu_launches++;
    a.pairs = b.key[1];
    a.part_cursor = b.part_cursor;
  }
  a.idx_out = b.idx[1]; a.sapos_out = b.sapos[1]; a.gd_out = b.gd[1];
  a.totals = b.totals;
  a.tiles = (m + RR_TILE - 1) / RR_TILE;
  BCE_TRY(c->desc.ensure(c, size_t(a.tiles) * 3 * sizeof(uint64_t)));
  a.desc = c->desc.as<uint64_t>();
  a.ticket = b.ticket;
  a.tag = uint32_t(next_tag(c));
  a.err = b.err;
  BCE_CUDA(c, cudaMemsetAsync(b.ticket, 0, 4, st));
  rerank_kernel<<<a.tiles, RR_THREADS, 0, st>>>(a);
  S.gpu_launches++;
  BCE_CUDA(c, cudaGetLastError());
  BCE_CUDA(c, cudaMemcpyAsync(b.rb->totals, b.totals, 8, cudaMemcpyDeviceToHost, st));
  BCE_CUDA(c, cudaMemcpyAsync(&b.rb->err, b.err, 4, cudaMemcpyDeviceToHost, st));
  float before = S.ms_rerank;
  BCE_TRY(lap(c, S.ms_rerank));
  BCE_TRACE("rerank round %d m=%u: %.3f ms (rank pairs partitioned=%d)", round, m, S.ms_rerank - before, int(p.binned));
  if (p.binned) {
    scatter_ranks_kernel<<<(m + 255) / 256, 256, 0, st>>>(b.key[1], m, b.rnk);
    S.gpu_launches++;
    BCE_CUDA(c, cudaGetLastError());
    before = S.ms_rerank;
    BCE_TRY(lap(c, S.ms_rerank));
    BCE_TRACE("rank scatter: %.3f ms", S.ms_rerank - before);
  }
  if (b.rb->err) { set_error(c, "suffix sort: chained-scan watchdog fired"); return BCE_GPU_E_INTERNAL; }
  *m_next = b.rb->totals[0];
  *groups = b.rb->totals[1];
  if (p.tiebreak && *m_next) { set_error(c, "suffix sort: ties left after index tie-break"); return BCE_GPU_E_INTERNAL; }
  return BCE_GPU_OK;
}

static int bwt_step(Ctx* c, const SortBuffers& b, uint32_t n, bool had_tiebreak) {
  cudaStream_t st = c->stream;
  const uint8_t* T = c->text.as<uint8_t>();
  uint8_t* L = c->bwt.as<uint8_t>();
  if (!had_tiebreak && n >= kBinnedBwtMinN) {
    const int shift = top_byte_shift(n);
    uint32_t* rows = reinterpret_cast<uint32_t*>(b.key[0]);
    BCE_TRACE("bwt binned shift=%d: positions binned through the inverse suffix array", shift);
    bwt_cursor_kernel<<<1, 256, 0, st>>>(b.part_cursor, shift);
    bwt_bin_kernel<<<(n + BG_TILE - 1) / BG_TILE, BG_THREADS, 0, st>>>(T, b.rnk, n, shift, b.part_cursor, rows);
    bwt_scatter_kernel<<<(n + 255) / 256, 256, 0, st>>>(rows, n, shift, L);
    c->stats.gpu_launches += 3;
  } else {
    BCE_TRACE("bwt gather: bytes gathered through the suffix array (tie-break ran: %d)", int(had_tiebreak));
    bwt_gather_kernel<<<((n + 3) / 4 + 255) / 256, 256, 0, st>>>(T, b.sa, n, L);
    c->stats.gpu_launches++;
  }
  BCE_CUDA(c, cudaGetLastError());
  BCE_CUDA(c, cudaMemcpyAsync(&b.rb->offset, b.sa, 4, cudaMemcpyDeviceToHost, st));
  BCE_TRY(lap(c, c->stats.ms_bwt_gather));
  c->offset = b.rb->offset;
  return BCE_GPU_OK;
}

int suffix_sort_bwt(Ctx* c, uint32_t n, uint32_t* sa_host) {
  BCE_TRY(c->bwt.ensure(c, size_t(n) + 64));
  SortBuffers b;
  BCE_TRY(carve(c, n, b));
  BCE_CUDA(c, cudaMemsetAsync(b.err, 0, 64, c->stream));
  bce_gpu_stats& S = c->stats;
  S.sort_rounds = 0;
  c->pass_ev_n = 0;

  BCE_CUDA(c, cudaEventRecord(c->ev[0], c->stream));
  pad_cyclic_kernel<<<1, 64, 0, c->stream>>>(c->text.as<uint8_t>(), n);
  S.gpu_launches++;
  BCE_CUDA(c, cudaGetLastError());
  BCE_TRY(lap(c, S.ms_pack));

  uint32_t m = n, groups = 0;
  uint64_t h = 8;
  bool had_tiebreak = false;
  for (int round = 0; m > 0; ++round) {
    if (round >= kMaxSortRounds) { set_error(c, "suffix sort: too many rounds"); return BCE_GPU_E_INTERNAL; }
    const RoundPlan p = plan_round(round, m, n, h, groups);
    had_tiebreak |= p.tiebreak;
    BCE_TRY(sort_round(c, b, p, round, m, n, h));
    BCE_TRY(rerank_round(c, b, p, round, m, n, &m, &groups));
    b.next_round();
    if (round > 0) h *= 2;
  }
  BCE_TRY(bwt_step(c, b, n, had_tiebreak));

  for (int i = 0; i + 1 < c->pass_ev_n; i += 2) {
    float pms = 0;
    if (cudaEventElapsedTime(&pms, c->pass_ev[i], c->pass_ev[i + 1]) == cudaSuccess) S.ms_radix_kernel += pms;
  }
  c->pass_ev_n = 0;
  c->bwt_resident = true;
  if (sa_host) BCE_TRY(d2h(c, sa_host, b.sa, size_t(n) * 4));
  return BCE_GPU_OK;
}

}
```

Before: 3626.

## Compress alphabet to 7-bit codes for round 0 and split rerank scan

Adds a preprocessing pass that maps byte values to dense codes when the alphabet has at most 128 symbols. Round-0 radix keys are then packed 7 bits per character, so only 7 digit passes are needed instead of 8, and the per-pass digit histograms are computed on the GPU from a pair histogram. Separately, the rerank stage's single-pass decoupled lookback scan is replaced by a heads kernel, a single-block carry scan and a non-atomic rerank kernel. This removes ticket and descriptor spinning but adds two extra launches per round and an extra code-text pass with a host sync.

```diff
diff --git a/bce_b200/csrc/api.cu b/bce_b200/csrc/api.cu
--- a/bce_b200/csrc/api.cu
+++ b/bce_b200/csrc/api.cu
@@ -262,6 +262,7 @@
   for (int i = 0; ok && i < 8; ++i) ok = cudaEventCreate(&c->ev[i]) == cudaSuccess;
   for (int i = 0; ok && i < 256; ++i) ok = cudaEventCreate(&c->pass_ev[i]) == cudaSuccess;
   if (ok) ok = bce::radix_init_device(c) == BCE_GPU_OK;
+  if (ok) ok = bce::sort_init_device(c) == BCE_GPU_OK;
   if (ok) ok = c->small.ensure(c, bce::kSmallBytes) == BCE_GPU_OK;
   if (ok) ok = c->pinned_small.ensure(c, bce::kSmallBytes) == BCE_GPU_OK;
   if (ok) ok = cudaStreamSynchronize(c->stream) == cudaSuccess;
diff --git a/bce_b200/csrc/common.cuh b/bce_b200/csrc/common.cuh
--- a/bce_b200/csrc/common.cuh
+++ b/bce_b200/csrc/common.cuh
@@ -81,6 +81,16 @@
   const uint64_t a = bswap64(T64[i >> 3]), b = bswap64(T64[(i >> 3) + 1]);
   const uint32_t sh = (i & 7u) * 8;
   return sh ? (a << sh) | (b >> (64 - sh)) : a;
+}
+
+__device__ __forceinline__ uint64_t pack_codes7(uint64_t w) {
+  w = (((w >> 8) & 0x007F007F007F007Full) << 7) | (w & 0x007F007F007F007Full);
+  w = (((w >> 16) & 0x00003FFF00003FFFull) << 14) | (w & 0x00003FFF00003FFFull);
+  return ((w >> 32) << 28) | (w & 0x0FFFFFFFull);
+}
+__device__ __forceinline__ uint64_t window_key_bits(const uint64_t* T64, uint32_t i, bool codes7) {
+  const uint64_t w = window_key(T64, i);
+  return codes7 ? pack_codes7(w) : w;
 }
 
 constexpr uint32_t kDescAgg = 1, kDescPrefix = 2;
@@ -181,35 +191,6 @@
   return excl;
 }
 
-__device__ __forceinline__ uint32_t lookback_warp_max(uint64_t* desc, uint32_t tile, uint32_t first,
-                                                      uint32_t tag, uint32_t agg, uint32_t* err) {
-  const unsigned lane = lane_id();
-  if (tile == first) {
-    if (lane == 0) desc_store(desc + tile, desc_pack(tag, kDescPrefix, agg));
-    return 0;
-  }
-  if (lane == 0) desc_store(desc + tile, desc_pack(tag, agg ? kDescPrefix : kDescAgg, agg));
-  uint32_t excl = 0;
-  int64_t base = int64_t(tile) - 1;
-  for (;;) {
-    int64_t t = base - lane;
-    bool inside = t >= int64_t(first);
-    uint64_t w = inside ? desc_wait(desc + t, tag, err) : desc_pack(tag, kDescPrefix, 0);
-    unsigned pm = __ballot_sync(0xffffffffu, desc_status(w) == kDescPrefix);
-    uint32_t v = uint32_t(w);
-    if (pm) {
-      unsigned stop = __ffs(pm) - 1;
-      if (lane > stop) v = 0;
-      excl = max(excl, __reduce_max_sync(0xffffffffu, v));
-      break;
-    }
-    excl = max(excl, __reduce_max_sync(0xffffffffu, v));
-    base -= 32;
-  }
-  if (lane == 0 && !agg) desc_store(desc + tile, desc_pack(tag, kDescPrefix, excl));
-  return excl;
-}
-
 template <int B>
 __device__ __forceinline__ uint32_t lookback_resolve_wide(uint64_t* desc, uint32_t tile, uint32_t first,
                                                           uint32_t tag, uint32_t agg, uint32_t* err) {
diff --git a/bce_b200/csrc/ctx.h b/bce_b200/csrc/ctx.h
--- a/bce_b200/csrc/ctx.h
+++ b/bce_b200/csrc/ctx.h
@@ -87,8 +87,7 @@
 constexpr size_t kSmallBase = kSmallHist + 8 * 256 * 4;
 constexpr size_t kSmallTicket = kSmallBase + 8 * 256 * 4;
 constexpr size_t kSmallErr = kSmallTicket + 64;
-constexpr size_t kSmallRerankTicket = kSmallErr + 64;
-constexpr size_t kSmallRerankTotals = kSmallRerankTicket + 64;
+constexpr size_t kSmallRerankTotals = kSmallErr + 64;
 constexpr size_t kSmallWavelet = kSmallRerankTotals + 64;
 constexpr size_t kSmallCse = kSmallWavelet + 2048;
 constexpr size_t kSmallUnbwt = kSmallCse + 1024;
@@ -100,6 +99,8 @@
 
 struct RadixHistSource {
   const uint8_t* window_text = nullptr;
+  bool codes7 = false;
+  bool host_hist = false;
   const uint32_t* dev_hist = nullptr;
   bool stable_first = false;
 };
@@ -126,6 +127,7 @@
 int h2d(Ctx* c, void* dst, const void* src, size_t bytes);
 int d2h(Ctx* c, void* dst, const void* src, size_t bytes);
 int radix_init_device(Ctx* c);
+int sort_init_device(Ctx* c);
 size_t scratch_budget(Ctx* c);
 
 }
diff --git a/bce_b200/csrc/radix_sort.cu b/bce_b200/csrc/radix_sort.cu
--- a/bce_b200/csrc/radix_sort.cu
+++ b/bce_b200/csrc/radix_sort.cu
@@ -59,6 +59,7 @@
   uint32_t* vout;
   uint32_t m;
   int shift;
+  bool codes7;
   const uint32_t* base;
   uint64_t* desc;
   uint32_t* ticket;
@@ -191,7 +192,7 @@
     const uint32_t idx = wbase + k * 32 + lane;
     const bool in = idx < p.m;
     if (FROM_TEXT) {
-      key[k] = in ? window_key(reinterpret_cast<const uint64_t*>(text), idx) : 0ull;
+      key[k] = in ? window_key_bits(reinterpret_cast<const uint64_t*>(text), idx, p.codes7) : 0ull;
       val[k] = idx;
     } else {
       key[k] = in ? p.kin[idx] : 0ull;
@@ -256,17 +257,10 @@
   const uint32_t* dev_hist = src ? src->dev_hist : nullptr;
   if (dev_hist == d_hist) BCE_CUDA(c, cudaMemsetAsync(d_base, 0, kSmallErr - kSmallBase, c->stream));
   else BCE_CUDA(c, cudaMemsetAsync(d_hist, 0, kSmallErr, c->stream));
-  if (dev_hist) {
+  if (src && src->host_hist) {
+  } else if (dev_hist) {
     BCE_CUDA(c, cudaMemcpyAsync(h_hist, dev_hist, npass * 256 * 4, cudaMemcpyDeviceToHost, c->stream));
     BCE_CUDA(c, cudaStreamSynchronize(c->stream));
-  } else if (window_text) {
-    byte_hist_launch(c, window_text, m, d_hist);
-    c->stats.gpu_launches++;
-    BCE_CUDA(c, cudaGetLastError());
-    BCE_CUDA(c, cudaMemcpyAsync(h_hist, d_hist, 256 * 4, cudaMemcpyDeviceToHost, c->stream));
-    BCE_CUDA(c, cudaStreamSynchronize(c->stream));
-    for (int p = npass - 1; p >= 0; --p)
-      for (int d = 0; d < 256; ++d) h_hist[p * 256 + d] = h_hist[d];
   } else {
     const size_t hsmem = size_t(RH_WARPS) * npass * 256 * 4;
     uint64_t hb64 = (uint64_t(m) + 255) / 256, hbmax = uint64_t(c->sm_count) * 3;
@@ -304,6 +298,7 @@
     RadixPass a;
     a.kin = kin; a.vin = vin; a.kout = kout; a.vout = vout;
     a.m = m; a.shift = shifts[p];
+    a.codes7 = src && src->codes7;
     a.base = d_base + p * 256;
     a.desc = c->desc.as<uint64_t>();
     a.ticket = d_ticket + p;
diff --git a/bce_b200/csrc/suffix_sort.cu b/bce_b200/csrc/suffix_sort.cu
--- a/bce_b200/csrc/suffix_sort.cu
+++ b/bce_b200/csrc/suffix_sort.cu
@@ -11,9 +11,54 @@
   if (k < 64) T[size_t(n) + k] = T[k % n];
 }
 
+struct CodeTable { uint8_t v[256]; };
+constexpr int kCodeBits = 7, kCodes = 1 << kCodeBits;
+constexpr size_t kPairHistSmem = size_t(kCodes) * kCodes * 4;
+
+__global__ void __launch_bounds__(256) code_text_kernel(const uint8_t* __restrict__ T, uint32_t n, CodeTable tab,
+                                                        uint8_t* __restrict__ C, uint32_t* __restrict__ pair_hist) {
+  extern __shared__ uint32_t s_pair[];
+  __shared__ uint8_t s_tab[256];
+  for (int i = threadIdx.x; i < kCodes * kCodes; i += blockDim.x) s_pair[i] = 0;
+  s_tab[threadIdx.x] = tab.v[threadIdx.x];
+  __syncthreads();
+  const uint32_t words = (n + 16 + 3) / 4;
+  const uint32_t* T32 = reinterpret_cast<const uint32_t*>(T);
+  uint32_t* C32 = reinterpret_cast<uint32_t*>(C);
+  for (uint32_t w = blockIdx.x * blockDim.x + threadIdx.x; w < words; w += gridDim.x * blockDim.x) {
+    const uint32_t t = T32[w];
+    uint32_t c[5];
+#pragma unroll
+    for (int j = 0; j < 4; ++j) c[j] = s_tab[(t >> (8 * j)) & 255u];
+    c[4] = s_tab[T[size_t(w) * 4 + 4]];
+    C32[w] = c[0] | (c[1] << 8) | (c[2] << 16) | (c[3] << 24);
+#pragma unroll
+    for (int j = 0; j < 4; ++j)
+      if (w * 4 + j < n) atomicAdd(&s_pair[(c[j] << kCodeBits) | c[j + 1]], 1u);
+  }
+  __syncthreads();
+  for (int i = threadIdx.x; i < kCodes * kCodes; i += blockDim.x)
+    if (s_pair[i]) atomicAdd(&pair_hist[i], s_pair[i]);
+}
+
+__global__ void __launch_bounds__(256) digit_hist_kernel(const uint32_t* __restrict__ pair_hist, uint32_t* __restrict__ hist) {
+  __shared__ uint32_t s_h[256];
+  const int p = blockIdx.x;
+  s_h[threadIdx.x] = 0;
+  __syncthreads();
+  for (int i = threadIdx.x; i < kCodes * kCodes; i += blockDim.x) {
+    const uint32_t v = pair_hist[i];
+    if (!v) continue;
+    const uint32_t x = uint32_t(i) >> kCodeBits, y = uint32_t(i) & (kCodes - 1);
+    atomicAdd(&s_h[((x & ((2u << p) - 1u)) << (kCodeBits - p)) | (y >> p)], v);
+  }
+  __syncthreads();
+  hist[p * 256 + threadIdx.x] = s_h[threadIdx.x];
+}
+
 constexpr int PK_ROWS = 8;
 
-__global__ void __launch_bounds__(256) pack_keys_kernel(const uint8_t* __restrict__ T, uint32_t n,
+__global__ void __launch_bounds__(256) pack_keys_kernel(const uint8_t* __restrict__ T, uint32_t n, bool codes7,
                                                         uint64_t* __restrict__ keys,
                                                         uint32_t* __restrict__ idx) {
   const uint64_t* T64 = reinterpret_cast<const uint64_t*>(T);
@@ -22,7 +67,7 @@
   for (int r = 0; r < PK_ROWS; ++r) {
     const uint32_t i = tile + r * 256 + threadIdx.x;
     if (i < n) {
-      keys[i] = window_key(T64, i);
+      keys[i] = window_key_bits(T64, i, codes7);
       idx[i] = i;
     }
   }
@@ -33,10 +78,119 @@
 constexpr int RR_ROWS = 16;
 constexpr int RR_WCHUNK = 32 * RR_ROWS;
 constexpr int RR_TILE = RR_WARPS * RR_WCHUNK;
-constexpr int RR_LOOKBACK = 4;
+constexpr int RR_CARRY_THREADS = 1024;
+
+__device__ __forceinline__ void rerank_row_masks(uint32_t H, uint32_t next_first, uint32_t rowbase, uint32_t m,
+                                                 uint32_t& S, uint32_t& SH, uint32_t& L) {
+  const uint32_t valid = rowbase >= m ? 0u : m - rowbase;
+  const uint32_t in_mask = valid >= 32u ? 0xFFFFFFFFu : (1u << valid) - 1u;
+  uint32_t nh = (H >> 1) | (next_first << 31);
+  if (valid <= 32u) nh |= valid ? ~((1u << (valid - 1u)) - 1u) : 0xFFFFFFFFu;
+  L = H & nh & in_mask;
+  S = in_mask & ~L;
+  SH = H & ~L;
+}
+
+__device__ __forceinline__ void rerank_warp_totals(const uint32_t (&H)[RR_ROWS], bool after_is_head, uint32_t wbase,
+                                                   uint32_t m, uint32_t& wsurv, uint32_t& wshead, uint32_t& whead) {
+  wsurv = wshead = whead = 0;
+#pragma unroll
+  for (int k = 0; k < RR_ROWS; ++k) {
+    uint32_t S, SH, L;
+    const uint32_t next_first = k + 1 < RR_ROWS ? (H[k + 1 < RR_ROWS ? k + 1 : k] & 1u) : (after_is_head ? 1u : 0u);
+    rerank_row_masks(H[k], next_first, wbase + k * 32, m, S, SH, L);
+    wsurv += __popc(S);
+    wshead += __popc(SH);
+    if (H[k]) whead = wbase + k * 32 + (31 - __clz(H[k])) + 1;
+  }
+}
+
+__global__ void __launch_bounds__(RR_THREADS) rerank_heads_kernel(const uint64_t* __restrict__ key, uint32_t m,
+                                                                  uint32_t* __restrict__ heads,
+                                                                  uint32_t* __restrict__ tsum, uint32_t tiles) {
+  __shared__ uint32_t s_w[3][RR_WARPS];
+  const unsigned tid = threadIdx.x, lane = tid & 31, warp = tid >> 5;
+  const uint32_t tile = blockIdx.x;
+  const uint32_t wbase = tile * RR_TILE + warp * RR_WCHUNK;
+  uint64_t k64[RR_ROWS];
+#pragma unroll
+  for (int k = 0; k < RR_ROWS; ++k) {
+    const uint32_t q = wbase + k * 32 + lane;
+    k64[k] = q < m ? key[q] : 0;
+  }
+  const uint64_t key_before = (wbase > 0 && wbase - 1 < m) ? key[wbase - 1] : 0;
+  const uint64_t key_after = (wbase + RR_WCHUNK < m) ? key[wbase + RR_WCHUNK] : 0;
+  uint32_t H[RR_ROWS], mine = 0;
+#pragma unroll
+  for (int k = 0; k < RR_ROWS; ++k) {
+    const uint32_t q = wbase + k * 32 + lane;
+    const uint64_t up = __shfl_up_sync(0xffffffffu, k64[k], 1);
+    const uint64_t wrap = k ? __shfl_sync(0xffffffffu, k64[k ? k - 1 : 0], 31) : key_before;
+    const uint64_t prev = lane ? up : wrap;
+    H[k] = __ballot_sync(0xffffffffu, q < m && (q == 0 || k64[k] != prev));
+    if (lane == unsigned(k)) mine = H[k];
+  }
+  const uint32_t row = wbase / 32 + lane;
+  if (lane < unsigned(RR_ROWS) && row * 32 < m) heads[row] = mine;
+  const bool after_is_head = (wbase + RR_WCHUNK >= m) || (key_after != __shfl_sync(0xffffffffu, k64[RR_ROWS - 1], 31));
+  uint32_t wsurv, wshead, whead;
+  rerank_warp_totals(H, after_is_head, wbase, m, wsurv, wshead, whead);
+  if (lane == 0) { s_w[0][warp] = whead; s_w[1][warp] = wsurv; s_w[2][warp] = wshead; }
+  __syncthreads();
+  if (tid < 3) {
+    uint32_t v = 0;
+#pragma unroll
+    for (int w = 0; w < RR_WARPS; ++w) v = tid ? v + s_w[tid][w] : max(v, s_w[0][w]);
+    tsum[size_t(tid) * tiles + tile] = v;
+  }
+}
+
+__global__ void __launch_bounds__(RR_CARRY_THREADS) rerank_carry_kernel(uint32_t* __restrict__ tsum, uint32_t tiles,
+                                                                        uint32_t* __restrict__ totals) {
+  constexpr int NW = RR_CARRY_THREADS / 32;
+  __shared__ uint32_t s_w[3][NW];
+  const unsigned lane = threadIdx.x & 31, warp = threadIdx.x >> 5;
+  uint32_t* th = tsum;
+  uint32_t* ts = tsum + tiles;
+  uint32_t* tg = tsum + 2 * size_t(tiles);
+  const uint32_t run = ((tiles + NW - 1) / NW + 31) & ~31u;
+  const uint32_t lo = min(tiles, warp * run), hi = min(tiles, lo + run);
+  uint32_t h = 0, s = 0, g = 0;
+  for (uint32_t j = lo + lane; j < hi; j += 32) { h = max(h, th[j]); s += ts[j]; g += tg[j]; }
+  h = __reduce_max_sync(0xffffffffu, h);
+  s = __reduce_add_sync(0xffffffffu, s);
+  g = __reduce_add_sync(0xffffffffu, g);
+  if (lane == 0) { s_w[0][warp] = h; s_w[1][warp] = s; s_w[2][warp] = g; }
+  __syncthreads();
+  uint32_t ch = 0, cs = 0, cg = 0;
+  for (unsigned w = 0; w < warp; ++w) { ch = max(ch, s_w[0][w]); cs += s_w[1][w]; cg += s_w[2][w]; }
+  if (threadIdx.x == RR_CARRY_THREADS - 1) { totals[0] = cs + s; totals[1] = cg + g; }
+  for (uint32_t base = lo; base < hi; base += 32) {
+    const uint32_t j = base + lane;
+    const bool in = j < hi;
+    const uint32_t vh = in ? th[j] : 0u, vs = in ? ts[j] : 0u, vg = in ? tg[j] : 0u;
+    uint32_t ih = vh, is = vs, ig = vg;
+#pragma unroll
+    for (int d = 1; d < 32; d <<= 1) {
+      const uint32_t oh = __shfl_up_sync(0xffffffffu, ih, d), os = __shfl_up_sync(0xffffffffu, is, d),
+                     og = __shfl_up_sync(0xffffffffu, ig, d);
+      if (lane >= unsigned(d)) { ih = max(ih, oh); is += os; ig += og; }
+    }
+    const uint32_t eh = __shfl_up_sync(0xffffffffu, ih, 1);
+    if (in) {
+      th[j] = max(ch, lane ? eh : 0u);
+      ts[j] = cs + is - vs;
+      tg[j] = cg + ig - vg;
+    }
+    ch = max(ch, __shfl_sync(0xffffffffu, ih, 31));
+    cs += __shfl_sync(0xffffffffu, is, 31);
+    cg += __shfl_sync(0xffffffffu, ig, 31);
+  }
+}
 
 struct RerankArgs {
-  const uint64_t* key;
+  const uint32_t* heads;
+  const uint32_t* carry;
   const uint32_t* idx;
   const uint32_t* sapos;
   uint32_t m;
@@ -48,40 +202,44 @@
   uint32_t* idx_out;
   uint32_t* sapos_out;
   uint32_t* gd_out;
-  uint32_t* totals;
-  uint64_t* desc;
   uint32_t tiles;
-  uint32_t* ticket;
-  uint32_t tag;
-  uint32_t* err;
 };
 
 __global__ void __launch_bounds__(RR_THREADS) rerank_kernel(RerankArgs a) {
   __shared__ uint32_t s_whead[RR_WARPS], s_wsurv[RR_WARPS], s_wshead[RR_WARPS];
-  __shared__ uint32_t s_tile;
-  __shared__ uint32_t s_carry[3];
   __shared__ uint32_t s_bcnt[256], s_bstart[256], s_gbase[256];
   __shared__ uint32_t s_bscan[RR_WARPS];
   __shared__ uint64_t s_stage[RR_TILE];
 
   const unsigned tid = threadIdx.x, lane = tid & 31, warp = tid >> 5;
-  if (tid == 0) s_tile = atomicAdd(a.ticket, 1u);
   s_bcnt[tid] = 0;
   __syncthreads();
-  const uint32_t tile = s_tile;
+  const uint32_t tile = blockIdx.x;
   const uint32_t wbase = tile * RR_TILE + warp * RR_WCHUNK;
   const bool binned = a.pairs != nullptr;
 
-  uint64_t key[RR_ROWS];
   uint32_t idx[RR_ROWS], sap[RR_ROWS];
 #pragma unroll
   for (int k = 0; k < RR_ROWS; ++k) {
     const uint32_t q = wbase + k * 32 + lane;
     const bool in = q < a.m;
-    key[k] = in ? a.key[q] : 0;
     idx[k] = in ? a.idx[q] : 0;
     sap[k] = in ? (a.sapos ? a.sapos[q] : q) : 0;
   }
+  uint32_t H[RR_ROWS];
+  const uint32_t rows = (a.m + 31) / 32, row0 = wbase / 32;
+#pragma unroll
+  for (int k = 0; k < RR_ROWS; k += 4) {
+    uint4 v = make_uint4(0, 0, 0, 0);
+    if (row0 + k + 3 < rows) v = *reinterpret_cast<const uint4*>(a.heads + row0 + k);
+    else if (row0 + k < rows) {
+      v.x = a.heads[row0 + k];
+      v.y = row0 + k + 1 < rows ? a.heads[row0 + k + 1] : 0u;
+      v.z = row0 + k + 2 < rows ? a.heads[row0 + k + 2] : 0u;
+    }
+    H[k] = v.x; H[k + 1] = v.y; H[k + 2] = v.z; H[k + 3] = v.w;
+  }
+  const bool after_is_head = (wbase + RR_WCHUNK >= a.m) || (a.heads[row0 + RR_ROWS] & 1u);
   uint32_t bpos[RR_ROWS / 2];
   if (binned) {
 #pragma unroll
@@ -91,40 +249,8 @@
       bpos[k / 2] = (k & 1) ? (bpos[k / 2] | (at << 16)) : at;
     }
   }
-  const uint64_t key_before = (wbase > 0 && wbase - 1 < a.m) ? a.key[wbase - 1] : 0;
-  const uint64_t key_after = (wbase + RR_WCHUNK < a.m) ? a.key[wbase + RR_WCHUNK] : 0;
-
-  uint32_t H[RR_ROWS];
-#pragma unroll
-  for (int k = 0; k < RR_ROWS; ++k) {
-    const uint32_t q = wbase + k * 32 + lane;
-    const uint64_t up = __shfl_up_sync(0xffffffffu, key[k], 1);
-    const uint64_t wrap = k ? __shfl_sync(0xffffffffu, key[k ? k - 1 : 0], 31) : key_before;
-    const uint64_t prev = lane ? up : wrap;
-    H[k] = __ballot_sync(0xffffffffu, q < a.m && (q == 0 || key[k] != prev));
-  }
-  const bool after_is_head = (wbase + RR_WCHUNK >= a.m) ||
-                             (key_after != __shfl_sync(0xffffffffu, key[RR_ROWS - 1], 31));
-  auto masks = [&](int k, uint32_t& S, uint32_t& SH, uint32_t& L) {
-    const uint32_t rowbase = wbase + k * 32;
-    const uint32_t valid = rowbase >= a.m ? 0u : a.m - rowbase;
-    const uint32_t in_mask = valid >= 32u ? 0xFFFFFFFFu : (1u << valid) - 1u;
-    const uint32_t next_first = k + 1 < RR_ROWS ? (H[k + 1 < RR_ROWS ? k + 1 : k] & 1u) : (after_is_head ? 1u : 0u);
-    uint32_t nh = (H[k] >> 1) | (next_first << 31);
-    if (valid <= 32u) nh |= valid ? ~((1u << (valid - 1u)) - 1u) : 0xFFFFFFFFu;
-    L = H[k] & nh & in_mask;
-    S = in_mask & ~L;
-    SH = H[k] & ~L;
-  };
-  uint32_t wsurv = 0, wshead = 0, whead = 0;
-#pragma unroll
-  for (int k = 0; k < RR_ROWS; ++k) {
-    uint32_t S, SH, L;
-    masks(k, S, SH, L);
-    wsurv += __popc(S);
-    wshead += __popc(SH);
-    if (H[k]) whead = wbase + k * 32 + (31 - __clz(H[k])) + 1;
-  }
+  uint32_t wsurv, wshead, whead;
+  rerank_warp_totals(H, after_is_head, wbase, a.m, wsurv, wshead, whead);
   if (lane == 0) { s_whead[warp] = whead; s_wsurv[warp] = wsurv; s_wshead[warp] = wshead; }
   __syncthreads();
   if (binned) {
@@ -133,33 +259,20 @@
     s_bstart[tid] = block_exclusive_scan<uint32_t, RR_THREADS>(c, s_bscan, tot);
     s_gbase[tid] = c ? atomicAdd(&a.part_cursor[tid], c) : 0u;
   }
-  uint32_t head_before = 0, surv_before = 0, shead_before = 0, tile_head = 0, tile_surv = 0, tile_shead = 0;
+  uint32_t run_head = a.carry[tile];
+  uint32_t out_at = a.carry[a.tiles + tile];
+  uint32_t gd_run = a.carry[2 * size_t(a.tiles) + tile];
 #pragma unroll
   for (int w = 0; w < RR_WARPS; ++w) {
-    const uint32_t hv = s_whead[w], sv = s_wsurv[w], shv = s_wshead[w];
-    if (unsigned(w) < warp) { head_before = max(head_before, hv); surv_before += sv; shead_before += shv; }
-    tile_head = max(tile_head, hv);
-    tile_surv += sv;
-    tile_shead += shv;
-  }
-  if (warp < 3) {
-    uint64_t* d = a.desc + size_t(warp) * a.tiles;
-    uint32_t v;
-    if (warp == 0) v = lookback_warp_max(d, tile, 0u, a.tag, tile_head, a.err);
-    else if (warp == 1) v = lookback_warp_wide<RR_LOOKBACK>(d, tile, 0u, a.tag, tile_surv, a.err);
-    else v = lookback_warp_wide<RR_LOOKBACK>(d, tile, 0u, a.tag, tile_shead, a.err);
-    if (lane == 0) s_carry[warp] = v;
-  }
-  __syncthreads();
-  uint32_t run_head = max(head_before, s_carry[0]);
-  uint32_t out_at = s_carry[1] + surv_before;
-  uint32_t gd_run = s_carry[2] + shead_before;
+    if (unsigned(w) < warp) { run_head = max(run_head, s_whead[w]); out_at += s_wsurv[w]; gd_run += s_wshead[w]; }
+  }
 
 #pragma unroll
   for (int k = 0; k < RR_ROWS; ++k) {
     const uint32_t q = wbase + k * 32 + lane;
     uint32_t S, SH, L;
-    masks(k, S, SH, L);
+    const uint32_t next_first = k + 1 < RR_ROWS ? (H[k + 1 < RR_ROWS ? k + 1 : k] & 1u) : (after_is_head ? 1u : 0u);
+    rerank_row_masks(H[k], next_first, wbase + k * 32, a.m, S, SH, L);
     const uint32_t le = lanemask_lt() | (1u << lane);
     const uint32_t hm = H[k] & le;
     const uint32_t my_head = hm ? wbase + k * 32 + (31 - __clz(hm)) + 1 : run_head;
@@ -188,10 +301,6 @@
       a.pairs[s_gbase[d] + (j - s_bstart[d])] = pr;
     }
   }
-  if (tile == a.tiles - 1 && tid == RR_THREADS - 1) {
-    a.totals[0] = s_carry[1] + tile_surv;
-    a.totals[1] = s_carry[2] + tile_shead;
-  }
 }
 
 __global__ void __launch_bounds__(256) partition_cursor_kernel(const uint32_t* __restrict__ hist, uint32_t* __restrict__ cursor) {
@@ -384,12 +493,12 @@
   int part_shift = 0;
 };
 
-static RoundPlan plan_round(int round, uint32_t m, uint32_t n, uint64_t h, uint32_t groups) {
+static RoundPlan plan_round(int round, uint32_t m, uint32_t n, uint64_t h, uint32_t groups, bool codes7) {
   RoundPlan p;
   p.binned = m >= kBinnedRanksMinSlots && size_t(n) * 4 > kBinnedRanksMinBytes;
   p.part_shift = top_byte_shift(n);
   if (round == 0) {
-    for (int s = 0; s < 64; s += 8) p.shifts[p.np++] = s;
+    for (int s = 0; s < (codes7 ? 8 * kCodeBits : 64); s += 8) p.shifts[p.np++] = s;
     return p;
   }
   p.tiebreak = h >= n;
@@ -419,7 +528,10 @@
   uint32_t* fb_idx[2];
   uint32_t* fb_slot;
   uint32_t *lt_pre, *lt_suf, *lt_cnt, *lt_off;
-  uint32_t *err, *ticket, *totals, *fb_total, *hist, *part_hist, *part_cursor;
+  uint32_t* rr_heads;
+  uint32_t* rr_tsum;
+  uint32_t* pair_hist;
+  uint32_t *err, *totals, *fb_total, *hist, *part_hist, *part_cursor;
   SortReadback* rb;
 
   void next_round() {
@@ -431,8 +543,10 @@
 
 static int carve(Ctx* c, uint32_t n, SortBuffers& b) {
   const size_t N = n, FB = N / kLocalFallbackDiv + 1, LT = N / LS_TILE + 2;
+  const size_t RH = (N + 31) / 32, RT = 3 * ((N + RR_TILE - 1) / RR_TILE);
   const size_t need = 2 * Carver::need(N, 8) + 8 * Carver::need(N, 4) + 2 * Carver::need(FB, 8) +
-                      3 * Carver::need(FB, 4) + 4 * Carver::need(LT, 4) + 4096;
+                      3 * Carver::need(FB, 4) + 4 * Carver::need(LT, 4) + Carver::need(RH, 4) + Carver::need(RT, 4) +
+                      Carver::need(kCodes * kCodes, 4) + 4096;
   BCE_TRY(c->scratch.ensure(c, need));
   Carver cv(c->scratch.p, c->scratch.cap);
   for (auto& k : b.key) k = cv.take<uint64_t>(N);
@@ -448,11 +562,13 @@
   b.lt_suf = cv.take<uint32_t>(LT);
   b.lt_cnt = cv.take<uint32_t>(LT);
   b.lt_off = cv.take<uint32_t>(LT);
+  b.rr_heads = cv.take<uint32_t>(RH);
+  b.rr_tsum = cv.take<uint32_t>(RT);
+  b.pair_hist = cv.take<uint32_t>(kCodes * kCodes);
   if (!cv.ok()) { set_error(c, "suffix sort: scratch carve failed"); return BCE_GPU_E_NOMEM; }
 
   char* small = c->small.as<char>();
   b.err = reinterpret_cast<uint32_t*>(small + kSmallErr);
-  b.ticket = reinterpret_cast<uint32_t*>(small + kSmallRerankTicket);
   b.totals = reinterpret_cast<uint32_t*>(small + kSmallRerankTotals);
   b.fb_total = b.totals + 3;
   b.hist = reinterpret_cast<uint32_t*>(small + kSmallHist);
@@ -472,10 +588,49 @@
   return BCE_GPU_OK;
 }
 
-static int sort_round(Ctx* c, SortBuffers& b, const RoundPlan& p, int round, uint32_t m, uint32_t n, uint64_t h) {
+static int round0_text(Ctx* c, SortBuffers& b, uint32_t n, const uint8_t** text, bool* codes7) {
+  cudaStream_t st = c->stream;
+  const uint8_t* T = c->text.as<uint8_t>();
+  uint32_t* h_hist = c->pinned_small.as<uint32_t>();
+  BCE_CUDA(c, cudaMemsetAsync(b.hist, 0, 256 * 4, st));
+  byte_hist_launch(c, T, n, b.hist);
+  c->stats.gpu_launches++;
+  BCE_CUDA(c, cudaGetLastError());
+  BCE_CUDA(c, cudaMemcpyAsync(h_hist, b.hist, 256 * 4, cudaMemcpyDeviceToHost, st));
+  BCE_CUDA(c, cudaStreamSynchronize(st));
+  CodeTable tab;
+  uint32_t sigma = 0;
+  for (int v = 0; v < 256; ++v) tab.v[v] = uint8_t(h_hist[v] ? sigma++ : 0);
+  *codes7 = sigma >= 2 && sigma <= uint32_t(kCodes);
+  BCE_TRACE("round 0: %u byte values, keys from %s", sigma, *codes7 ? "7-bit codes" : "bytes");
+  if (!*codes7) {
+    *text = T;
+    for (int p = 7; p >= 0; --p)
+      for (int d = 0; d < 256; ++d) h_hist[p * 256 + d] = h_hist[d];
+    return BCE_GPU_OK;
+  }
+  uint8_t* C = reinterpret_cast<uint8_t*>(b.rnk);
+  BCE_CUDA(c, cudaMemsetAsync(b.pair_hist, 0, kPairHistSmem, st));
+  const uint32_t words = (n + 16 + 3) / 4, want = (words + 255) / 256, most = uint32_t(c->sm_count) * 3;
+  code_text_kernel<<<want < most ? want : most, 256, kPairHistSmem, st>>>(T, n, tab, C, b.pair_hist);
+  digit_hist_kernel<<<kCodeBits, 256, 0, st>>>(b.pair_hist, b.hist);
+  c->stats.gpu_launches += 2;
+  BCE_CUDA(c, cudaGetLastError());
+  BCE_CUDA(c, cudaMemcpyAsync(h_hist, b.hist, kCodeBits * 256 * 4, cudaMemcpyDeviceToHost, st));
+  BCE_CUDA(c, cudaStreamSynchronize(st));
+  *text = C;
+  return BCE_GPU_OK;
+}
+
+int sort_init_device(Ctx* c) {
+  BCE_CUDA(c, cudaFuncSetAttribute(code_text_kernel, cudaFuncAttributeMaxDynamicSharedMemorySize, int(kPairHistSmem)));
+  return BCE_GPU_OK;
+}
+
+static int sort_round(Ctx* c, SortBuffers& b, const RoundPlan& p, int round, uint32_t m, uint32_t n, uint64_t h,
+                      const uint8_t* text0, bool codes7) {
   cudaStream_t st = c->stream;
   bce_gpu_stats& S = c->stats;
-  const uint8_t* T = c->text.as<uint8_t>();
   const uint32_t second_h = uint32_t(p.tiebreak ? 0 : h);
   const uint32_t ltiles = (m + LS_TILE - 1) / LS_TILE;
   bool local = false;
@@ -542,7 +697,8 @@
     S.sort_fallback_elems += m_fb;
   } else {
     RadixHistSource src;
-    if (round == 0) src.window_text = T; else src.dev_hist = b.hist;
+    if (round == 0) { src.window_text = text0; src.codes7 = codes7; src.host_hist = true; }
+    else src.dev_hist = b.hist;
     uint64_t* ks; uint32_t* vs;
     BCE_TRY(radix_sort_pairs(c, b.key[0], b.key[1], b.idx[0], b.idx[1], m, p.shifts, p.np, &ks, &vs, &ran, &src));
     if (ks != b.key[0]) {
@@ -550,7 +706,7 @@
       std::swap(b.idx[0], b.idx[1]);
     }
     if (round == 0 && ran == 0) {
-      pack_keys_kernel<<<(n + 256 * PK_ROWS - 1) / (256 * PK_ROWS), 256, 0, st>>>(T, n, b.key[0], b.idx[0]);
+      pack_keys_kernel<<<(n + 256 * PK_ROWS - 1) / (256 * PK_ROWS), 256, 0, st>>>(text0, n, codes7, b.key[0], b.idx[0]);
       S.gpu_launches++;
     }
   }
@@ -567,7 +723,12 @@
   cudaStream_t st = c->stream;
   bce_gpu_stats& S = c->stats;
   RerankArgs a;
-  a.key = b.key[0]; a.idx = b.idx[0]; a.sapos = round ? b.sapos[0] : nullptr; a.m = m;
+  a.tiles = (m + RR_TILE - 1) / RR_TILE;
+  rerank_heads_kernel<<<a.tiles, RR_THREADS, 0, st>>>(b.key[0], m, b.rr_heads, b.rr_tsum, a.tiles);
+  rerank_carry_kernel<<<1, RR_CARRY_THREADS, 0, st>>>(b.rr_tsum, a.tiles, b.totals);
+  S.gpu_launches += 2;
+  BCE_CUDA(c, cudaGetLastError());
+  a.heads = b.rr_heads; a.carry = b.rr_tsum; a.idx = b.idx[0]; a.sapos = round ? b.sapos[0] : nullptr; a.m = m;
   a.sa = b.sa; a.rnk = b.rnk;
   a.pairs = nullptr; a.part_cursor = nullptr; a.part_shift = p.part_shift;
   if (p.binned) {
@@ -584,14 +745,6 @@
     a.part_cursor = b.part_cursor;
   }
   a.idx_out = b.idx[1]; a.sapos_out = b.sapos[1]; a.gd_out = b.gd[1];
-  a.totals = b.totals;
-  a.tiles = (m + RR_TILE - 1) / RR_TILE;
-  BCE_TRY(c->desc.ensure(c, size_t(a.tiles) * 3 * sizeof(uint64_t)));
-  a.desc = c->desc.as<uint64_t>();
-  a.ticket = b.ticket;
-  a.tag = uint32_t(next_tag(c));
-  a.err = b.err;
-  BCE_CUDA(c, cudaMemsetAsync(b.ticket, 0, 4, st));
   rerank_kernel<<<a.tiles, RR_THREADS, 0, st>>>(a);
   S.gpu_launches++;
   BCE_CUDA(c, cudaGetLastError());
@@ -654,14 +807,19 @@
   BCE_CUDA(c, cudaGetLastError());
   BCE_TRY(lap(c, S.ms_pack));
 
+  const uint8_t* text0 = nullptr;
+  bool codes7 = false;
+  BCE_TRY(round0_text(c, b, n, &text0, &codes7));
+  BCE_TRY(lap(c, S.ms_radix));
+
   uint32_t m = n, groups = 0;
   uint64_t h = 8;
   bool had_tiebreak = false;
   for (int round = 0; m > 0; ++round) {
     if (round >= kMaxSortRounds) { set_error(c, "suffix sort: too many rounds"); return BCE_GPU_E_INTERNAL; }
-    const RoundPlan p = plan_round(round, m, n, h, groups);
+    const RoundPlan p = plan_round(round, m, n, h, groups, codes7);
     had_tiebreak |= p.tiebreak;
-    BCE_TRY(sort_round(c, b, p, round, m, n, h));
+    BCE_TRY(sort_round(c, b, p, round, m, n, h, text0, codes7));
     BCE_TRY(rerank_round(c, b, p, round, m, n, &m, &groups));
     b.next_round();
     if (round > 0) h *= 2;
```

New measurement: 3757, median of 6. 1.04x the previous value.
